# SebTanz/StochQuant

Measured on AMD Instinct MI355X. Metric: lattice-site Langevin updates/sec at 256³ fp32; achieved HBM GB/s vs peak, higher is better.
Workload: dtype fp32

## Files before the change

### stochquant_amd/build.py

```python
import argparse
import concurrent.futures as cf
import hashlib
import os
import shutil
import subprocess
import sys

PKG = os.path.dirname(os.path.abspath(__file__))
ROOT = os.path.dirname(PKG)
CSRC = os.path.join(PKG, "csrc")
OBJ = os.path.join(PKG, "_obj")
LIBDIR = os.path.join(PKG, "lib")
BINDIR = os.path.join(PKG, "bin")
LIB = os.path.join(LIBDIR, "libstochquant.so")
TAUHOST = os.path.join(BINDIR, "tauhost.o")
ROCM = os.environ.get("ROCM_PATH", "/opt/rocm")
HIPCC = os.path.join(ROCM, "bin", "hipcc")
ARCH = os.environ.get("SQ_OFFLOAD_ARCH", "gfx950")

DEVICE_SOURCES = ["sq_phi4.hip", "sq_phi4_run.hip", "sq_qm1d.hip", "sq_qm1d_ens.hip", "sq_qm1d_gs.hip", "sq_phi4_ens.hip",
                  "sq_selftest.hip", "sq_p2p.hip", "sq_fields.hip"]
HOST_SOURCES = ["sq_core.cpp", "sq_comm.cpp", "sq_phi4_create.cpp", "sq_phi4_plan.cpp", "sq_phi4_steps.cpp",
                "sq_phi4_frames.cpp", "sq_phi4_fields.cpp", "sq_qm1d_host.cpp", "sq_ens.cpp", "sq_phi4_ens.cpp",
                "sq_diag.cpp", "sq_io.cpp"]
HEADERS = ["sq_internal.h", "sq_ctx.h", "sq_rng.h", "sq_dpp.h", "sq_glibcf.h", "sq_ens.h", "sq_phi4_ens.h", "sq_qm1d_math.h"]
INCLUDES = {"sq_phi4_run.hip": ["sq_phi4.hip"], "sq_phi4_ens.hip": ["sq_phi4.hip"]}
COMMON = ["-O3", "-fPIC", "-std=c++17", "-ffp-contract=off", "-fno-slp-vectorize", "-Wall",
          "-Wno-unused-function"]


def _digest(paths, extra):
    h = hashlib.sha256()
    for p in paths:
        with open(p, "rb") as fh:
            h.update(fh.read())
    h.update(" ".join(extra).encode())
    return h.hexdigest()


def build_id(objs):
    def h(paths):
        d = hashlib.sha256()
        for p in paths:
            with open(p, "rb") as fh:
                d.update(fh.read())
        return d.hexdigest()[:16]
    phi4 = [o for o in objs if os.path.basename(o) == "sq_phi4.hip.o"]
    return f"phi4:{h(phi4)} lib:{h(objs)}"


def _run(cmd):
    r = subprocess.run(cmd, capture_output=True, text=True)
    if r.returncode != 0:
        raise RuntimeError("build failed:\n" + " ".join(cmd) + "\n" + r.stdout + r.stderr)
    return r


def build(force=False, verbose=False):
    os.makedirs(OBJ, exist_ok=True)
    os.makedirs(LIBDIR, exist_ok=True)
    os.makedirs(BINDIR, exist_ok=True)
    hdrs = [os.path.join(CSRC, h) for h in HEADERS] + [os.path.join(ROOT, "include", "stochquant.h")]
    jobs = []
    for src in DEVICE_SOURCES + HOST_SOURCES:
        s = os.path.join(CSRC, src)
        o = os.path.join(OBJ, src + ".o")
        flags = COMMON + [f"--offload-arch={ARCH}", "-x", "hip"]
        stamp = o + ".sha"
        dig = _digest([s] + [os.path.join(CSRC, d) for d in INCLUDES.get(src, [])] + hdrs, flags)
        if not force and os.path.exists(o) and os.path.exists(stamp) and open(stamp).read() == dig:
            continue
        jobs.append(([HIPCC] + flags + ["-c", s, "-o", o], stamp, dig))
    with cf.ThreadPoolExecutor(max_workers=min(8, os.cpu_count() or 4)) as ex:
        for (cmd, stamp, dig), _ in zip(jobs, ex.map(lambda j: _run(j[0]), jobs)):
            with open(stamp, "w") as fh:
                fh.write(dig)
            if verbose:
                print(" ".join(cmd))
    objs = [os.path.join(OBJ, s + ".o") for s in DEVICE_SOURCES + HOST_SOURCES]
    bid = build_id(objs)
    bid_obj = os.path.join(OBJ, "sq_build_id.cpp.o")
    bid_stamp = bid_obj + ".sha"
    if jobs or force or not os.path.exists(bid_obj) or not os.path.exists(bid_stamp) or \
            open(bid_stamp).read() != bid:
        _run([HIPCC] + COMMON + ["-x", "c++", f'-DSQ_BUILD_ID="{bid}"', "-c",
                                 os.path.join(CSRC, "sq_build_id.cpp"), "-o", bid_obj])
        with open(bid_stamp, "w") as fh:
            fh.write(bid)
        jobs.append(None)
    if jobs or force or not os.path.exists(LIB):
        _run([HIPCC, f"--offload-arch={ARCH}", "-shared", "-fPIC", "-o", LIB] + objs + [bid_obj]
             + [f"-L{ROCM}/lib", "-lrccl", f"-Wl,-rpath,{ROCM}/lib"])
    th_src = os.path.join(CSRC, "tauhost.cpp")
    if jobs or force or not os.path.exists(TAUHOST) or \
            os.path.getmtime(th_src) > os.path.getmtime(TAUHOST):
        _run(["g++", "-O2", "-std=c++17", "-Wall", "-o", TAUHOST, th_src,
              f"-L{LIBDIR}", "-lstochquant", "-Wl,-rpath,$ORIGIN/../lib", f"-Wl,-rpath,{ROCM}/lib", "-lm"])
    root_link = os.path.join(ROOT, "tauhost.o")
    try:
        if os.path.islink(root_link) or os.path.exists(root_link):
            os.remove(root_link)
        os.symlink(os.path.relpath(TAUHOST, ROOT), root_link)
    except OSError:
        shutil.copy2(TAUHOST, root_link)
    return LIB


def build_oracle(verbose=False):
    odir = os.path.join(ROOT, "oracle")
    r = subprocess.run(["make", "-C", odir, "-j4"], capture_output=True, text=True)
    if r.returncode != 0:
        raise RuntimeError("oracle build failed:\n" + r.stdout + r.stderr)
    if verbose:
        print(r.stdout)
    return os.path.join(odir, "liboracle.so")


def main(argv=None):
    ap = argparse.ArgumentParser()
    ap.add_argument("--force", action="store_true")
    ap.add_argument("-v", "--verbose", action="store_true")
    a = ap.parse_args(argv)
    print(build(force=a.force, verbose=a.verbose))
    print(build_oracle(verbose=a.verbose))


if __name__ == "__main__":
    sys.exit(main())
```

### stochquant_amd/csrc/sq_internal.h

```cpp
#pragma once
#include <hip/hip_runtime.h>
#include <stdint.h>

#include <string>

namespace sq {

int set_error(int code, const std::string &msg);

}

struct sq_ctx;

namespace sq {

struct FrameState {
    float T, V;
    int init;
    int stab_cnt;
};
int frame_state_get(const sq_ctx *c, FrameState *fs);
int frame_state_set(sq_ctx *c, const FrameState &fs);

struct FrameCtl;
struct FrameFoldArgs {
    const FrameCtl *cin;
    FrameCtl *cout;
    const unsigned long long *md;
    const unsigned int *am;
    const int *flag;
    float *rec;
    int *stable_out;
    double *dtau_out;
    const float *snap;
    int L;
};
struct RecClear {
    unsigned long long *md;
    unsigned int *am;
    int *flag;
    int n;
};
constexpr int kFoldMaxL = 64;

struct Phi4StepArgs {
    const float *in;
    float *out;
    int Lx, Ly, nz, gz;
    int zlo, zhi, zstep, zc, nzc;
    int nzr, zlen;
    int periodic;
    int nxseg, nyg, nunits;
    long long zg0;
    long long Lzg;
    float h, m2, lam6, sig, clampv;
    float sigq;
    int fin;
    uint32_t k0, k1, s_lo, s_hi;
    int *flag;
    unsigned long long *st_md;
    unsigned int *st_a;
    float *snap;
    const float *dcoef;
    int prio;
    unsigned long long *stamps;
    FrameFoldArgs fold;
    RecClear clr;
    float *buf0, *buf1, *buf2;
    const FrameCtl *tctl;
    int tk;
    int tspec;
    const unsigned int *gate;
    unsigned int gate_seq;
    int n_reg, tzc, tlen, tlo0, thi0, ntz;
    int *gate_err;
};
constexpr int kStabSlots = 32;

struct FrameCtl {
    double dtau;
    double C;
    float coef[4];
    float T, V;
    int stab_cnt;
    int adapt;
    int stable;
    int fired;
    int flag;
    int frames;
    int tri, bs, bw0, bw1, nl_odd;
};
struct FrameEndArgs {
    const FrameCtl *cin;
    FrameCtl *cout;
    const unsigned long long *md;
    const unsigned int *am;
    const int *flag;
    unsigned long long *md_next;
    unsigned int *am_next;
    int *flag_next;
    int L;
    float *rec;
    int *stable_out;
    double *dtau_out;
    float4 *dst;
    const float4 *snap;
    long long n4;
};
hipError_t phi4_frame_end_launch(const FrameEndArgs &e, hipStream_t s);
constexpr double kSqrt2Ln2 = 1.1774100225154747;

struct Phi4Geom {
    int qx;
    int r;
    int wy;
    int pf;
    int v;
};

bool phi4_tb2_supported(int Lx, int Ly);
hipError_t phi4_tb2_launch(const Phi4StepArgs &a, hipStream_t s, hipEvent_t start = nullptr,
                           hipEvent_t stop = nullptr, uint64_t *kid = nullptr);

struct Tb2RunArgs {
    unsigned int *flags;
    int *err;
    unsigned int base;
    int npairs;
    unsigned long long *stamps;
};
bool phi4_tb2_run_ok(const Phi4StepArgs &a, int dev);
hipError_t phi4_tb2_run_launch(const Phi4StepArgs &a, const Tb2RunArgs &r, hipStream_t s, hipEvent_t start = nullptr,
                               hipEvent_t stop = nullptr, uint64_t *kid = nullptr);
void phi4_run_kernel_id_name(uint64_t kid, char *name, size_t cap);

struct Tb2StageArgs {
    float *stage;
    int G;
    unsigned int *ctr;
};
bool phi4_tb2_stage_ok(const Phi4StepArgs &a, int G);
hipError_t phi4_tb2_stage_launch(const Phi4StepArgs &a, const Tb2StageArgs &g, hipStream_t s,
                                 hipEvent_t start = nullptr, hipEvent_t stop = nullptr, uint64_t *kid = nullptr);

void phi4_kernel_id_name(uint64_t kid, char *name, size_t cap);
inline unsigned phi4_kernel_id_grid(uint64_t kid) { return (unsigned)(kid >> 32); }

bool phi4_geometry(int Lx, int Ly, Phi4Geom *g);
void phi4_fill_units(Phi4StepArgs &a, const Phi4Geom &g);
hipError_t phi4_step_launch(const Phi4StepArgs &a, const Phi4Geom &g, hipStream_t s,
                            hipEvent_t start = nullptr, hipEvent_t stop = nullptr, uint64_t *kid = nullptr);
hipError_t phi4_init_hash_launch(float *slab, int Lx, int Ly, int nz, long long zg0, unsigned long long key,
                                 double amp, hipStream_t s);
hipError_t phi4_init_launch(float *slab, int Lx, int Ly, int nz, long long zg0, uint32_t k0,
                            uint32_t k1, float amp, hipStream_t s);
constexpr int kMomBlocks = 1024;
hipError_t phi4_moments_launch(const float *slab, long long n, double *acc, unsigned int *acc_max, double *part,
                               hipStream_t s);
hipError_t phi4_slices_launch(const float *slab, int Lx, int Ly, int nz, double *out,
                              hipStream_t s);

enum class P2pRed { kMaxU32, kMaxI32, kMaxU64, kMaxF64, kSumF64 };
hipError_t p2p_handshake_launch(unsigned int *up_from_dn, unsigned int *dn_from_up, const unsigned int *from_dn,
                                const unsigned int *from_up, unsigned int e, unsigned int polls, int *err,
                                hipStream_t s, const unsigned int *pre = nullptr, unsigned int pre_n = 0);
hipError_t p2p_copy2_launch(float *d0, const float *s0, float *d1, const float *s1, size_t n, hipStream_t s);
hipError_t p2p_fold_launch(const unsigned char *slots, int nranks, size_t cap, void *out, size_t n, P2pRed red,
                           hipStream_t s);

struct Qm1dState {
    double omega_in;
    double omega_out;
    double lrgVl;
    int lrgEl;
    int stable;
    int steps_done;
    int sync_error;
};

struct Qm1dArgs {
    const double *f, *x, *xx0;
    double *nf, *nx, *nxx0;
    double *fs, *xs, *ds;
    double *om;
    float *xi, *tcl;
    double *dd;
    Qm1dState *st;
    int N, pot, loops, runs;
    double a, a2, h, sig, sigw, kconst;
    uint32_t k0, k1;
    unsigned long long tick;
    int gbar;
    unsigned int bar_polls;
    int bar_skip;
    unsigned long long *dbg;
};

int qm1d_sites_per_thread(int N);
constexpr int kQm1dMaxN = 1024 * 64;
constexpr int kQm1dRegMaxN = 4096;
constexpr int kQm1dGridAux = 2048;
constexpr int kQm1dStampBlocks = kQm1dMaxN / 512;
constexpr size_t kQm1dTableCap = size_t(16) << 30;
hipError_t qm1d_frame_launch(const Qm1dArgs &a, hipStream_t s);
hipError_t qm1d_prep_launch(const Qm1dArgs &a, hipStream_t s);

struct Qm1dGsState {
    double omega_in, omega_out, lrgVl;
    int lrgEl, stable, steps_done;
    int rows_ready;
    long long consumed;
    int sync_error;
    int brk_step, brk_item;
    int pad;
};

struct Qm1dGsArgs {
    const double *f0, *x0, *xx00;
    double *nf, *nx, *nxx0;
    double *nfp;
    const double *xi;
    double *om;
    double *xc;
    void *cand;
    int *flags;
    int tag;
    double *hist;
    Qm1dGsState *st;
    int N, pot, loops, runs;
    double a, a2, h, sig, sigw, kconst;
};

constexpr int kQm1dGsMaxN = 4096;
int qm1d_gs_block(int N);
constexpr int kLcgChunks = 16384;
constexpr size_t kLcgScratch = 3 * (size_t)kLcgChunks + 1;
hipError_t qm1d_gs_lcg_launch(unsigned long long seed, int N, long long ncalls, uint32_t *w1,
                              uint32_t *w2, unsigned long long *seeds, double *xi,
                              unsigned long long *scr, hipStream_t s);
size_t qm1d_gs_cand_bytes(int loops);
hipError_t qm1d_gs_frame_launch(const Qm1dGsArgs &a, hipStream_t s);

hipError_t selftest_normals_launch(float *out, size_t nquads, unsigned long long quad0,
                                   uint32_t stream, unsigned long long step, uint32_t k0,
                                   uint32_t k1, hipStream_t s);
hipError_t selftest_dpp_launch(float *out, hipStream_t s);
hipError_t selftest_dpp_mix_launch(int mode, int blocks, int iters, unsigned *errs, float *sink, hipStream_t s);
hipError_t selftest_philox_launch(const uint32_t *ck, uint32_t *out, hipStream_t s);
hipError_t selftest_libm_launch(int fn, const float *x, float *y, long long n, hipStream_t s);
hipError_t selftest_bm_tables_launch(float *t, hipStream_t s);
hipError_t copy_launch(const float4 *in, float4 *out, size_t n4, bool nt, hipStream_t s);

}
```

### stochquant_amd/csrc/sq_phi4.hip

```cpp
#include <hip/hip_ext.h>

#include <algorithm>
#include <cstdio>
#include <cstring>

#include "sq_dpp.h"
#include "sq_internal.h"
#include "sq_rng.h"

namespace sq {

namespace {

typedef float f32x4v __attribute__((ext_vector_type(4)));

__device__ __forceinline__ float from_left_lane(float v) {
    return __builtin_bit_cast(float, __builtin_amdgcn_mov_dpp(__builtin_bit_cast(int, v), 0x13C, 0xF, 0xF, true));
}
__device__ __forceinline__ float from_right_lane(float v) {
    return __builtin_bit_cast(float, __builtin_amdgcn_mov_dpp(__builtin_bit_cast(int, v), 0x134, 0xF, 0xF, true));
}
__device__ __forceinline__ float from_left_lane_or(float v, float edge) {
    return __builtin_bit_cast(float, __builtin_amdgcn_update_dpp(__builtin_bit_cast(int, edge),
                                                                 __builtin_bit_cast(int, v), 0x138, 0xF, 0xF, false));
}
__device__ __forceinline__ float from_right_lane_or(float v, float edge) {
    return __builtin_bit_cast(float, __builtin_amdgcn_update_dpp(__builtin_bit_cast(int, edge),
                                                                 __builtin_bit_cast(int, v), 0x130, 0xF, 0xF, false));
}

__device__ __forceinline__ __amdgpu_buffer_rsrc_t plane_rsrc(const float *base, int padded,
                                                             size_t plane, uint32_t pbytes) {
    return __builtin_amdgcn_make_buffer_rsrc((void *)(base + (size_t)padded * plane), (short)0,
                                             (int)pbytes, 0x00020000);
}
template <int LAUX = 0>
__device__ __forceinline__ float4 bload4(__amdgpu_buffer_rsrc_t r, uint32_t off, uint32_t soff = 0) {
    const f32x4v v = __builtin_amdgcn_raw_buffer_load_b128(r, off, soff, LAUX);
    return make_float4(v.x, v.y, v.z, v.w);
}
template <int AUX = 0>
__device__ __forceinline__ void bstore4(__amdgpu_buffer_rsrc_t r, uint32_t off, float4 v) {
    const uint32_t soff = 0;
    const f32x4v w = {v.x, v.y, v.z, v.w};
    __builtin_amdgcn_raw_buffer_store_b128(w, r, off, soff, AUX);
}
template <int LAUX = 0>
__device__ __forceinline__ float bload1(__amdgpu_buffer_rsrc_t r, uint32_t off, uint32_t soff = 0) {
    return __builtin_bit_cast(float, __builtin_amdgcn_raw_buffer_load_b32(r, off, soff, LAUX));
}

__device__ __forceinline__ int padded_index(const Phi4StepArgs &A, int zl) {
    if (A.periodic) {
        if (zl < 0) return A.nz;
        if (zl >= A.nz) return 1;
    }
    return zl + A.gz;
}

__device__ __forceinline__ int global_z(const Phi4StepArgs &A, int zl) {
    const int Lz = (int)A.Lzg;
    int zg = (int)A.zg0 + zl;
    if (zg < 0) zg += Lz;
    else if (zg >= Lz) zg -= Lz;
    return zg;
}

template <bool NZ>
__device__ __forceinline__ float site_update(float phi, float xm, float xp, float ym, float yp,
                                             float zm, float zp, float xi, const Phi4StepArgs &A) {
    const float nb = ((xm + xp) + (ym + yp)) + (zm + zp);
    const float lap = __builtin_fmaf(-6.0f, phi, nb);
    const float g = __builtin_fmaf(A.lam6, phi * phi, A.m2);
    const float drift = __builtin_fmaf(-phi, g, lap);
    const float det = __builtin_fmaf(A.h, drift, phi);
    const float v = NZ ? __builtin_fmaf(A.sigq, xi, det) : det;
    return fmaxf(fminf(v, A.clampv), -A.clampv);
}

typedef float f32x2 __attribute__((ext_vector_type(2)));
template <bool NZ>
__device__ __forceinline__ float4 site_update4(float4 c, float lft, float rgt, float4 up, float4 dn,
                                               float4 zm, float4 zp, const f32x4n &xi,
                                               const Phi4StepArgs &A, bool fin, f32x2 m2v,
                                               float *mpre = nullptr) {
    const f32x2 c0 = {c.x, c.y}, c1 = {c.z, c.w};
    float s02, s13;
    asm("v_add_f32 %0, %1, %2" : "=v"(s02) : "v"(c.x), "v"(c.z));
    asm("v_add_f32 %0, %1, %2" : "=v"(s13) : "v"(c.y), "v"(c.w));
    const f32x2 x0 = {lft + c.y, s02}, x1 = {s13, c.z + rgt};
    const f32x2 y0 = f32x2{up.x, up.y} + f32x2{dn.x, dn.y}, y1 = f32x2{up.z, up.w} + f32x2{dn.z, dn.w};
    const f32x2 z0 = f32x2{zm.x, zm.y} + f32x2{zp.x, zp.y}, z1 = f32x2{zm.z, zm.w} + f32x2{zp.z, zp.w};
    const f32x2 nb0 = (x0 + y0) + z0, nb1 = (x1 + y1) + z1;
    const f32x2 m6 = {-6.0f, -6.0f}, l6 = {A.lam6, A.lam6}, m2 = m2v, h = {A.h, A.h};
    const f32x2 lap0 = __builtin_elementwise_fma(m6, c0, nb0), lap1 = __builtin_elementwise_fma(m6, c1, nb1);
    const f32x2 g0 = __builtin_elementwise_fma(l6, c0 * c0, m2), g1 = __builtin_elementwise_fma(l6, c1 * c1, m2);
    const f32x2 d0 = __builtin_elementwise_fma(-c0, g0, lap0), d1 = __builtin_elementwise_fma(-c1, g1, lap1);
    f32x2 v0 = __builtin_elementwise_fma(h, d0, c0), v1 = __builtin_elementwise_fma(h, d1, c1);
    if (NZ) {
        const f32x2 sg = {A.sigq, A.sigq};
        v0 = __builtin_elementwise_fma(sg, f32x2{xi.a, xi.b}, v0);
        v1 = __builtin_elementwise_fma(sg, f32x2{xi.c, xi.d}, v1);
    }
    const float cl = A.clampv;
    float4 o = make_float4(v0.x, v0.y, v1.x, v1.y);
    const float m = fmaxf(fmaxf(fmaxf(fabsf(o.x), fabsf(o.y)), fabsf(o.z)), fabsf(o.w));
    float mo = m;
    if (!fin || !(m < cl)) {
        o = make_float4(fmaxf(fminf(o.x, cl), -cl), fmaxf(fminf(o.y, cl), -cl), fmaxf(fminf(o.z, cl), -cl),
                        fmaxf(fminf(o.w, cl), -cl));
        if (mpre != nullptr) mo = fmaxf(fmaxf(fabsf(o.x), fabsf(o.y)), fmaxf(fabsf(o.z), fabsf(o.w)));
    }
    if (mpre != nullptr) *mpre = mo;
    return o;
}

struct FrameAcc {
    float m, d;
    float mw;
    float am;
};
__device__ __forceinline__ FrameAcc frame_acc() {
    return FrameAcc{-__builtin_inff(), 0.f, -__builtin_inff(), 0.f};
}

__device__ __forceinline__ float vmax(float a, float b) {
    float r;
    asm("v_max_f32 %0, %1, %2" : "=v"(r) : "v"(a), "v"(b));
    return r;
}
__device__ __forceinline__ float vmax3(float a, float b, float c) {
    float r;
    asm("v_max3_f32 %0, %1, %2, %3" : "=v"(r) : "v"(a), "v"(b), "v"(c));
    return r;
}

__device__ __forceinline__ void stab_site(FrameAcc &f, float o, float c, float xi, float sig) {
    const float dn = fabsf(__builtin_fmaf(-sig, xi, o - c));
    const float dt = vmax(f.d, dn);
    const bool gt = o > f.m, eq = o == f.m;
    const float d1 = eq ? dt : f.d;
    f.d = gt ? dn : d1;
    f.m = vmax(f.m, o);
}

template <bool NZ, bool BW = false>
__device__ __forceinline__ void frame_sites(const Phi4StepArgs &A, FrameAcc &f, const float4 &o, const float4 &c,
                                            const f32x4n &xi, float *bw = nullptr, bool pre = false,
                                            float mpre = 0.f) {
    const float mo = pre ? mpre : fmaxf(fmaxf(fabsf(o.x), fabsf(o.y)), fmaxf(fabsf(o.z), fabsf(o.w)));
    f.am = vmax(f.am, mo);
    {
        if (__ballot(mo >= f.mw) == 0ull) return;
        const float o4 = vmax(vmax3(o.x, o.y, o.z), o.w);
        if (__ballot(o4 >= f.mw) == 0ull) return;
        if constexpr (BW) {
            f.mw = vmax(f.mw, __hip_atomic_load(bw, __ATOMIC_RELAXED, __HIP_MEMORY_SCOPE_WORKGROUP));
        }
        if (!BW || __ballot(o4 >= f.mw) != 0ull) {
            const float s = NZ ? A.sigq : 0.f;
            stab_site(f, o.x, c.x, xi.a, s);
            stab_site(f, o.y, c.y, xi.b, s);
            stab_site(f, o.z, c.z, xi.c, s);
            stab_site(f, o.w, c.w, xi.d, s);
            f.mw = dpp_all_max_f(f.m);
            if (BW && (threadIdx.x & 63) == 0)
                __hip_atomic_fetch_max(bw, f.mw, __ATOMIC_RELAXED, __HIP_MEMORY_SCOPE_WORKGROUP);
        }
    }
}

__device__ __forceinline__ uint32_t ord_f32(float v) {
    const uint32_t u = __float_as_uint(v);
    return (u & 0x80000000u) ? ~u : (u | 0x80000000u);
}

__device__ __forceinline__ void frame_flush(const Phi4StepArgs &A, const FrameAcc &f, int rec, uint64_t *sk,
                                            uint32_t *sa) {
    const bool bad = f.am >= A.clampv;
    if (__ballot(bad) != 0ull && (threadIdx.x & 63) == 0) atomicOr(A.flag, 1);
    if (A.st_md == nullptr) return;
    uint64_t k = dpp_all_max_u64(((uint64_t)ord_f32(f.m) << 32) | __float_as_uint(f.d));
    uint32_t a = (uint32_t)dpp_all_max_i((int)__float_as_uint(fminf(f.am, A.clampv)));
    const int w = threadIdx.x >> 6, nw = blockDim.x >> 6;
    __syncthreads();
    if ((threadIdx.x & 63) == 0) {
        sk[w] = k;
        sa[w] = a;
    }
    __syncthreads();
    if (threadIdx.x == 0) {
        for (int i = 1; i < nw; ++i) {
            k = sk[i] > k ? sk[i] : k;
            a = sa[i] > a ? sa[i] : a;
        }
        const int slot = rec * kStabSlots + (int)(blockIdx.x % kStabSlots);
        atomicMax(A.st_md + slot, (unsigned long long)k);
        atomicMax(A.st_a + slot, a);
    }
}

__device__ __forceinline__ void frame_flush2(const Phi4StepArgs &A, const FrameAcc &f1, const FrameAcc &f2,
                                             unsigned long long *fk, uint32_t *fa) {
    const bool bad = f1.am >= A.clampv || f2.am >= A.clampv;
    if (__ballot(bad) != 0ull && (threadIdx.x & 63) == 0) atomicOr(A.flag, 1);
    if (A.st_md == nullptr) return;
    if (f1.m >= f1.mw && f1.mw > -__builtin_inff())
        atomicMax(&fk[0], ((uint64_t)ord_f32(f1.m) << 32) | __float_as_uint(f1.d));
    if (f2.m >= f2.mw && f2.mw > -__builtin_inff())
        atomicMax(&fk[1], ((uint64_t)ord_f32(f2.m) << 32) | __float_as_uint(f2.d));
    const uint32_t a1 = (uint32_t)dpp_all_max_i((int)__float_as_uint(fminf(f1.am, A.clampv)));
    const uint32_t a2 = (uint32_t)dpp_all_max_i((int)__float_as_uint(fminf(f2.am, A.clampv)));
    if ((threadIdx.x & 63) == 0) {
        atomicMax(&fa[0], a1);
        atomicMax(&fa[1], a2);
    }
    __syncthreads();
    if (threadIdx.x < 2) {
        const int slot = (int)threadIdx.x * kStabSlots + (int)(blockIdx.x % kStabSlots);
        atomicMax(A.st_md + slot, fk[threadIdx.x]);
        atomicMax(A.st_a + slot, fa[threadIdx.x]);
    }
}

__device__ __forceinline__ uint32_t uni(uint32_t v) { return __builtin_amdgcn_readfirstlane(v); }

template <int R>
__device__ __forceinline__ void philox_field(u32x4 (&c)[R], uint32_t k0, uint32_t k1) {
    const uint32_t cy = c[0].y, cz = c[0].z, cw = c[0].w;
    const uint64_t p1u = (uint64_t)kPhiloxM1 * cz;
    const uint32_t u0 = uni((uint32_t)(p1u >> 32) ^ cy ^ k0), u1 = uni((uint32_t)p1u);
    const uint32_t a0 = cw ^ k1;
    uint32_t n2[R], n3[R];
#pragma unroll
    for (int r = 0; r < R; ++r) {
        const uint64_t p0 = (uint64_t)kPhiloxM0 * c[r].x;
        n2[r] = (uint32_t)(p0 >> 32) ^ a0;
        n3[r] = (uint32_t)p0;
    }
    k0 += kPhiloxW0;
    k1 += kPhiloxW1;
    const uint64_t p0u = (uint64_t)kPhiloxM0 * u0;
    const uint32_t b0 = uni(u1 ^ k0), b2 = uni((uint32_t)(p0u >> 32) ^ k1), u3 = uni((uint32_t)p0u);
#pragma unroll
    for (int r = 0; r < R; ++r) {
        const uint64_t p1 = (uint64_t)kPhiloxM1 * n2[r];
        c[r] = u32x4{(uint32_t)(p1 >> 32) ^ b0, (uint32_t)p1, b2 ^ n3[r], u3};
    }
    k0 += kPhiloxW0;
    k1 += kPhiloxW1;
    const uint32_t d2 = uni(u3 ^ k1);
#pragma unroll
    for (int r = 0; r < R; ++r) {
        const uint64_t p0 = (uint64_t)kPhiloxM0 * c[r].x;
        const uint64_t p1 = (uint64_t)kPhiloxM1 * c[r].z;
        const uint32_t n0 = __builtin_amdgcn_bitop3_b32((uint32_t)(p1 >> 32), c[r].y, k0, 0x96);
        c[r] = u32x4{n0, (uint32_t)p1, (uint32_t)(p0 >> 32) ^ d2, (uint32_t)p0};
    }
#pragma unroll
    for (int rnd = 3; rnd < 10; ++rnd) {
        k0 += kPhiloxW0;
        k1 += kPhiloxW1;
#pragma unroll
        for (int r = 0; r < R; ++r) {
            const uint64_t p0 = (uint64_t)kPhiloxM0 * c[r].x;
            const uint64_t p1 = (uint64_t)kPhiloxM1 * c[r].z;
            const uint32_t n0 = __builtin_amdgcn_bitop3_b32((uint32_t)(p1 >> 32), c[r].y, k0, 0x96);
            const uint32_t m2 = __builtin_amdgcn_bitop3_b32((uint32_t)(p0 >> 32), c[r].w, k1, 0x96);
            c[r] = u32x4{n0, (uint32_t)p1, m2, (uint32_t)p0};
        }
    }
}

template <int R>
__device__ __forceinline__ void philox_rows(u32x4 (&c)[R], uint32_t k0, uint32_t k1) {
#pragma unroll
    for (int rnd = 0; rnd < 10; ++rnd) {
        if (rnd) {
            k0 += kPhiloxW0;
            k1 += kPhiloxW1;
        }
#pragma unroll
        for (int r = 0; r < R; ++r) {
            const uint64_t p0 = (uint64_t)kPhiloxM0 * c[r].x;
            const uint64_t p1 = (uint64_t)kPhiloxM1 * c[r].z;
            const uint32_t n0 = __builtin_amdgcn_bitop3_b32((uint32_t)(p1 >> 32), c[r].y, k0, 0x96);
            const uint32_t n2 = __builtin_amdgcn_bitop3_b32((uint32_t)(p0 >> 32), c[r].w, k1, 0x96);
            c[r] = u32x4{n0, (uint32_t)p1, n2, (uint32_t)p0};
        }
    }
}

template <int R, int V>
struct Slot {
    float4 row[R * V];
    float4 hm[V], hp[V];
};

template <int QX, int R, int V>
struct Lane {
    uint32_t voff[R * V];
    uint32_t vm[V], vp[V];
    uint32_t vl[R], vr[R];
    uint32_t qoff[R * V];
    bool rows_ok;
    int lane;
};

template <int QX, int R, int V>
__device__ __forceinline__ void load_slot(const Phi4StepArgs &A, const Lane<QX, R, V> &L,
                                          Slot<R, V> &s, int zl, bool halo, size_t plane,
                                          uint32_t pbytes) {
    const __amdgpu_buffer_rsrc_t rs = plane_rsrc(A.in, padded_index(A, zl), plane, pbytes);
#pragma unroll
    for (int k = 0; k < R * V; ++k) s.row[k] = bload4(rs, L.voff[k]);
    if (halo) {
#pragma unroll
        for (int v = 0; v < V; ++v) {
            s.hm[v] = bload4(rs, L.vm[v]);
            s.hp[v] = bload4(rs, L.vp[v]);
        }
    }
}

template <int QX, int R, int V, bool MS, bool NZ, bool PK, int SAUX, bool FR>
__device__ __forceinline__ void plane_compute(const Phi4StepArgs &A, const Lane<QX, R, V> &L,
                                              const Slot<R, V> &P, const Slot<R, V> &C,
                                              const Slot<R, V> &N, int z, size_t plane,
                                              uint32_t pbytes, uint32_t qplane, uint32_t slo, uint32_t shi,
                                              FrameAcc &fa) {
    float el[R], er[R];
    if constexpr (MS) {
        const __amdgpu_buffer_rsrc_t rs = plane_rsrc(A.in, padded_index(A, z), plane, pbytes);
#pragma unroll
        for (int r = 0; r < R; ++r) {
            el[r] = 0.f;
            er[r] = 0.f;
            if (L.lane == 0) el[r] = bload1(rs, L.vl[r]);
            if (L.lane == 63) er[r] = bload1(rs, L.vr[r]);
        }
    }
    f32x4n xi[R * V];
    if constexpr (NZ) {
        u32x4 c[R * V];
        const uint32_t qbase = (uint32_t)global_z(A, z) * qplane;
#pragma unroll
        for (int k = 0; k < R * V; ++k) c[k] = u32x4{qbase + L.qoff[k], kStreamField << 24, slo, shi};
        philox_field<R * V>(c, A.k0, A.k1);
#pragma unroll
        for (int k = 0; k < R * V; ++k) {
            box_muller_q(c[k].x, c[k].y, xi[k].a, xi[k].b);
            box_muller_q(c[k].z, c[k].w, xi[k].c, xi[k].d);
        }
    } else {
#pragma unroll
        for (int k = 0; k < R * V; ++k) xi[k] = f32x4n{0.f, 0.f, 0.f, 0.f};
    }
    float4 hmv[V], hpv[V];
#pragma unroll
    for (int v = 0; v < V; ++v) {
        hmv[v] = C.hm[v];
        hpv[v] = C.hp[v];
    }
    const __amdgpu_buffer_rsrc_t ws = plane_rsrc(A.out, A.periodic ? z + 1 : z + A.gz, plane, pbytes);
#pragma unroll
    for (int r = 0; r < R; ++r) {
        float rl[V], rr[V];
#pragma unroll
        for (int v = 0; v < V; ++v) {
            const float4 cc = C.row[r * V + v];
            if constexpr (QX == 64) {
                rl[v] = from_left_lane(cc.w);
                rr[v] = from_right_lane(cc.x);
            } else {
                const int seg = L.lane & ~(QX - 1), xq = L.lane & (QX - 1);
                rl[v] = __shfl(cc.w, seg | ((xq + QX - 1) & (QX - 1)), 64);
                rr[v] = __shfl(cc.x, seg | ((xq + 1) & (QX - 1)), 64);
            }
        }
#pragma unroll
        for (int v = 0; v < V; ++v) {
            const int k = r * V + v;
            const float4 cc = C.row[k];
            const float4 up = r > 0 ? C.row[r > 0 ? k - V : 0] : hmv[v];
            const float4 dn = r < R - 1 ? C.row[r < R - 1 ? k + V : 0] : hpv[v];
            float lft = rl[v], rgt = rr[v];
            if constexpr (V > 1) {
                if (L.lane == 0) lft = rl[(v + V - 1) % V];
                if (L.lane == 63) rgt = rr[(v + 1) % V];
            }
            if constexpr (MS) {
                if (v == 0 && L.lane == 0) lft = el[r];
                if (v == V - 1 && L.lane == 63) rgt = er[r];
            }
            float4 o;
            if constexpr (PK) {
                o = site_update4<NZ>(cc, lft, rgt, up, dn, P.row[k], N.row[k], xi[k], A, A.fin != 0,
                                     f32x2{A.m2, A.m2});
            } else {
                o.x = site_update<NZ>(cc.x, lft, cc.y, up.x, dn.x, P.row[k].x, N.row[k].x, xi[k].a, A);
                o.y = site_update<NZ>(cc.y, cc.x, cc.z, up.y, dn.y, P.row[k].y, N.row[k].y, xi[k].b, A);
                o.z = site_update<NZ>(cc.z, cc.y, cc.w, up.z, dn.z, P.row[k].z, N.row[k].z, xi[k].c, A);
                o.w = site_update<NZ>(cc.w, cc.z, rgt, up.w, dn.w, P.row[k].w, N.row[k].w, xi[k].d, A);
            }
            if constexpr (FR) frame_sites<NZ>(A, fa, o, cc, xi[k]);
            if (L.rows_ok) bstore4<SAUX>(ws, L.voff[k], o);
        }
    }
}

template <int QX, int R, int V, bool MS, bool NZ, bool PK, int SAUX, bool FR>
__device__ __forceinline__ void plane_step(const Phi4StepArgs &A, const Lane<QX, R, V> &L,
                                           const Slot<R, V> &P, const Slot<R, V> &C, Slot<R, V> &N,
                                           int z, int zend, size_t plane, uint32_t pbytes,
                                           uint32_t qplane, uint32_t slo, uint32_t shi, FrameAcc &fa) {
    load_slot<QX, R, V>(A, L, N, z + 1, z + 1 < zend, plane, pbytes);
    plane_compute<QX, R, V, MS, NZ, PK, SAUX, FR>(A, L, P, C, N, z, plane, pbytes, qplane, slo, shi, fa);
}

template <int QX, int R, int V, bool MS, bool NZ, int PF, bool FR>
__device__ __forceinline__ void unit_run(const Phi4StepArgs &A, int unit, FrameAcc &fa, uint32_t slo, uint32_t shi) {
    constexpr int RS = 64 / QX;
    const int xs = unit % A.nxseg;
    const int rest = unit / A.nxseg;
    const int yg = rest % A.nyg;
    const int zk = rest / A.nyg;
    const int zbeg = A.zlo + zk * A.zstep;
    const int zend = min(zbeg + A.zc, A.zhi);

    const int Lx = A.Lx, Ly = A.Ly;
    const size_t plane = (size_t)Lx * (size_t)Ly;
    const uint32_t pbytes = (uint32_t)(plane * sizeof(float));
    const uint32_t qplane = (uint32_t)(plane >> 2);
    Lane<QX, R, V> L;
    L.lane = threadIdx.x & 63;
    const int xq = L.lane & (QX - 1);
    const int rsid = L.lane / QX;
    const int xspan = xs * (4 * QX * V);
    const int x = xspan + 4 * xq;
    const int y0r = yg * (RS * R) + rsid * R;
    L.rows_ok = y0r < Ly;
    const int y0 = L.rows_ok ? y0r : 0;
    const int ym = y0 == 0 ? Ly - 1 : y0 - 1;
    const int yp = (y0 + R == Ly) ? 0 : y0 + R;
    const int xl = (xspan == 0 ? Lx : xspan) - 1;
    const int xr = (xspan + 4 * QX * V == Lx) ? 0 : xspan + 4 * QX * V;
#pragma unroll
    for (int r = 0; r < R; ++r) {
#pragma unroll
        for (int v = 0; v < V; ++v) {
            const int xv = x + 4 * QX * v;
            L.voff[r * V + v] = (uint32_t)(((y0 + r) * Lx + xv) * 4);
            L.qoff[r * V + v] = (uint32_t)(((y0 + r) * Lx + xv) >> 2);
        }
        L.vl[r] = (uint32_t)(((y0 + r) * Lx + xl) * 4);
        L.vr[r] = (uint32_t)(((y0 + r) * Lx + xr) * 4);
    }
#pragma unroll
    for (int v = 0; v < V; ++v) {
        L.vm[v] = (uint32_t)((ym * Lx + x + 4 * QX * v) * 4);
        L.vp[v] = (uint32_t)((yp * Lx + x + 4 * QX * v) * 4);
    }

    Slot<R, V> S0, S1, S2;
    load_slot<QX, R, V>(A, L, S0, zbeg - 1, false, plane, pbytes);
    load_slot<QX, R, V>(A, L, S1, zbeg, true, plane, pbytes);
    constexpr bool PK = PF >= 3;
    constexpr int SAUX = PF == 4 ? 2 : PF == 7 ? 17 : 0;
    for (int z = zbeg; z < zend; z += 3) {
        plane_step<QX, R, V, MS, NZ, PK, SAUX, FR>(A, L, S0, S1, S2, z, zend, plane, pbytes, qplane, slo, shi, fa);
        if (z + 1 >= zend) break;
        plane_step<QX, R, V, MS, NZ, PK, SAUX, FR>(A, L, S1, S2, S0, z + 1, zend, plane, pbytes, qplane, slo, shi, fa);
        if (z + 2 >= zend) break;
        plane_step<QX, R, V, MS, NZ, PK, SAUX, FR>(A, L, S2, S0, S1, z + 2, zend, plane, pbytes, qplane, slo, shi, fa);
    }
}

__device__ __forceinline__ uintptr_t pick_buf(const Phi4StepArgs &A, int i) {
    const uintptr_t b0 = reinterpret_cast<uintptr_t>(A.buf0), b1 = reinterpret_cast<uintptr_t>(A.buf1),
                    b2 = reinterpret_cast<uintptr_t>(A.buf2);
    return i == 0 ? b0 : (i == 1 ? b1 : b2);
}

__device__ __forceinline__ float unord_f32_dev(uint32_t o);
__device__ __forceinline__ void frame_decide(FrameCtl &c, float T, float V, int fired, int flag);

struct FrameOv {
    uintptr_t in, out, snap;
    float h, sig, sigq;
};

template <bool FR>
__device__ __forceinline__ void frame_fold(const Phi4StepArgs &A, FrameOv &ov) {
    if constexpr (FR) {
        if (A.clr.md != nullptr) {
            const int gt = (int)(blockIdx.x * blockDim.x + threadIdx.x), gs = (int)(gridDim.x * blockDim.x);
            for (int q = gt; q < A.clr.n; q += gs) {
                A.clr.md[q] = 0ull;
                A.clr.am[q] = 0u;
            }
            if (gt == 0) *A.clr.flag = 0;
        }
        if (A.fold.cin == nullptr) return;
        __shared__ unsigned long long sK[kFoldMaxL];
        __shared__ unsigned int sAm[kFoldMaxL];
        __shared__ float sCoef[3];
        __shared__ int sSt, sBuf[2];
        const int L = A.fold.L;
        for (int j = (int)threadIdx.x; j < L; j += (int)blockDim.x) {
            sK[j] = 0ull;
            sAm[j] = 0u;
        }
        __syncthreads();
        for (int q = (int)threadIdx.x; q < L * kStabSlots; q += (int)blockDim.x) {
            atomicMax(&sK[q / kStabSlots], A.fold.md[q]);
            atomicMax(&sAm[q / kStabSlots], A.fold.am[q]);
        }
        __syncthreads();
        if (threadIdx.x == 0) {
            FrameCtl c = *A.fold.cin;
            float T = c.T, V = c.V;
            int fired = -1;
            for (int j = 0; j < L; ++j) {
                const float M = unord_f32_dev((uint32_t)(sK[j] >> 32)), D = __uint_as_float((uint32_t)sK[j]);
                const float Aj = __uint_as_float(sAm[j]);
                const bool f = M > T && D > V;
                T = M;
                V = V < Aj ? Aj : V;
                if (f) {
                    fired = j;
                    break;
                }
            }
            frame_decide(c, T, V, fired, *A.fold.flag);
            sCoef[0] = c.coef[0];
            sCoef[1] = c.coef[1];
            sCoef[2] = c.coef[2];
            sSt = c.stable;
            sBuf[0] = c.bs;
            sBuf[1] = c.bw0;
            if (blockIdx.x == 0) {
                *A.fold.cout = c;
                if (A.fold.stable_out) *A.fold.stable_out = c.stable;
                if (A.fold.dtau_out) *A.fold.dtau_out = c.dtau;
            }
        }
        if (blockIdx.x == 0)
            for (int j = (int)threadIdx.x; j < L; j += (int)blockDim.x) {
                A.fold.rec[j] = unord_f32_dev((uint32_t)(sK[j] >> 32));
                A.fold.rec[L + j] = __uint_as_float((uint32_t)sK[j]);
                A.fold.rec[2 * L + j] = __uint_as_float(sAm[j]);
            }
        __syncthreads();
        const bool tri = A.buf0 != nullptr, st = sSt != 0;
        const uintptr_t snapv = reinterpret_cast<uintptr_t>(A.fold.snap) -
                                sizeof(float) * (size_t)A.gz * (size_t)A.Lx * (size_t)A.Ly;
        const uintptr_t in = tri ? pick_buf(A, sBuf[0]) : (st ? ov.in : snapv);
        const uintptr_t out = tri ? pick_buf(A, sBuf[1]) : ov.out;
        const uintptr_t sn = (!tri && !st) ? uintptr_t(0) : ov.snap;
        ov.in = in;
        ov.out = out;
        ov.snap = sn;
        ov.h = sCoef[0];
        ov.sig = sCoef[1];
        ov.sigq = sCoef[2];
    }
}

struct TriCheck {
    uintptr_t in, out;
    bool on;
};

template <bool FR, bool SPEC = false>
__device__ __forceinline__ Phi4StepArgs frame_args(const Phi4StepArgs &A0, TriCheck *chk = nullptr) {
    if constexpr (FR) {
        FrameOv ov{reinterpret_cast<uintptr_t>(A0.in), reinterpret_cast<uintptr_t>(A0.out),
                   reinterpret_cast<uintptr_t>(A0.snap), A0.h, A0.sig, A0.sigq};
        if (A0.dcoef != nullptr) {
            ov.h = A0.dcoef[0];
            ov.sig = A0.dcoef[1];
            ov.sigq = A0.dcoef[2];
        }
        if (A0.tctl != nullptr) {
            const int bs = A0.tctl->bs, bw0 = A0.tctl->bw0, bw1 = A0.tctl->bw1;
            const int bi = A0.tk == 0 ? bs : ((A0.tk & 1) ? bw0 : bw1);
            const int bo = A0.tk == 0 ? bw0 : ((A0.tk & 1) ? bw1 : bw0);
            const uintptr_t in = pick_buf(A0, bi), out = pick_buf(A0, bo);
            if (SPEC && A0.tspec != 0) {
                chk->in = in;
                chk->out = out;
                chk->on = true;
            } else {
                ov.in = in;
                ov.out = out;
            }
        }
        frame_fold<FR>(A0, ov);
        Phi4StepArgs A = A0;
        A.in = reinterpret_cast<const float *>(ov.in);
        A.out = reinterpret_cast<float *>(ov.out);
        A.snap = reinterpret_cast<float *>(ov.snap);
        A.h = ov.h;
        A.sig = ov.sig;
        A.sigq = ov.sigq;
        return A;
    } else {
        return A0;
    }
}

template <int QX, int R, int V, bool MS, bool NZ, int PF, bool FR>
__global__ __launch_bounds__(256) void phi4_step_kernel(const Phi4StepArgs A0) {
    const Phi4StepArgs A = frame_args<FR>(A0);
    const int nb = gridDim.x, b = blockIdx.x;
    const int lb = (nb & 7) == 0 ? (b & 7) * (nb >> 3) + (b >> 3) : b;
    const int unit = __builtin_amdgcn_readfirstlane(lb * 4 + (int)(threadIdx.x >> 6));
    FrameAcc fa = frame_acc();
    if (unit < A.nunits) unit_run<QX, R, V, MS, NZ, PF, FR>(A, unit, fa, A.s_lo, A.s_hi);
    if constexpr (FR) {
        __shared__ uint64_t sk[4];
        __shared__ uint32_t sa[4];
        frame_flush(A, fa, 0, sk, sa);
    }
}

__device__ __forceinline__ void block_stamp(const Phi4StepArgs &A, int at) {
    const unsigned long long rt = __builtin_amdgcn_s_memrealtime(), ct = __builtin_amdgcn_s_memtime();
    A.stamps[2 * blockIdx.x + at] = rt;
    A.stamps[2 * gridDim.x + 2 * blockIdx.x + at] = ct;
}
__device__ __forceinline__ void block_end_stamp(const Phi4StepArgs &A) {
    if (A.stamps == nullptr) return;
    __syncthreads();
    if (threadIdx.x == 0) block_stamp(A, 1);
}

struct PrioQ {
    int t0, t1, t2;
    __device__ __forceinline__ PrioQ(int z0, int span)
        : t0(z0 - 1 + (span + 3) / 4), t1(z0 - 1 + (2 * span + 3) / 4), t2(z0 - 1 + (3 * span + 3) / 4) {}
    __device__ __forceinline__ int q(int p) const { return (p >= t0) + (p >= t1) + (p >= t2); }
};

__device__ __forceinline__ void prio_by_progress(int q) {
    switch (q) {
    case 0: __builtin_amdgcn_s_setprio(3); break;
    case 1: __builtin_amdgcn_s_setprio(2); break;
    case 2: __builtin_amdgcn_s_setprio(1); break;
    default: __builtin_amdgcn_s_setprio(0); break;
    }
}

struct TbBlock {
    int yb, xs, z0, z1;
    bool gated;
};
template <bool WIDE>
__device__ __forceinline__ TbBlock tb_block(const Phi4StepArgs &A, int b, int nb) {
    TbBlock t;
    t.gated = A.gate != nullptr && b >= A.n_reg;
    const int nbr = A.gate != nullptr ? A.n_reg : nb;
    const int lb = t.gated ? b - A.n_reg : ((nbr & 7) == 0 ? (b & 7) * (nbr >> 3) + (b >> 3) : b);
    t.yb = lb % A.nyg;
    const int rest = lb / A.nyg;
    t.xs = WIDE ? rest % A.nxseg : 0;
    const int zk = WIDE ? rest / A.nxseg : rest;
    if (t.gated) {
        const int r0 = zk >= A.ntz ? A.thi0 : A.tlo0;
        t.z0 = r0 + (zk % A.ntz) * A.tzc;
        t.z1 = min(t.z0 + A.tzc, r0 + A.tlen);
    } else {
        const int r0 = A.zlo + (zk / A.nzr) * A.zstep;
        t.z0 = r0 + (zk % A.nzr) * A.zc;
        t.z1 = min(t.z0 + A.zc, r0 + A.zlen);
    }
    return t;
}

constexpr unsigned int kGateSpinMax = 1u << 24;
__device__ __forceinline__ bool tb_gate_wait(const Phi4StepArgs &A) {
    __shared__ int s_gate_ok;
    if (threadIdx.x == 0) {
        unsigned int n = 0;
        int ok = 1;
        while (__hip_atomic_load(A.gate, __ATOMIC_ACQUIRE, __HIP_MEMORY_SCOPE_AGENT) < A.gate_seq) {
            __builtin_amdgcn_s_sleep(2);
            if (++n >= kGateSpinMax) {
                if (A.gate_err) __hip_atomic_fetch_or(A.gate_err, 1, __ATOMIC_RELAXED, __HIP_MEMORY_SCOPE_AGENT);
                ok = 0;
                break;
            }
        }
        s_gate_ok = ok;
    }
    __syncthreads();
    __builtin_amdgcn_fence(__ATOMIC_ACQUIRE, "agent");
    return s_gate_ok != 0;
}

constexpr int kTbRows = 8;
constexpr int kTbWaves = kTbRows + 2;

__device__ __forceinline__ int tb_pidx(const Phi4StepArgs &A, int zl) {
    if (A.periodic) zl = zl < 0 ? zl + A.nz : (zl >= A.nz ? zl - A.nz : zl);
    return zl + A.gz;
}

template <bool NZ>
__device__ __forceinline__ f32x4n tb_noise(const Phi4StepArgs &A, uint32_t qz, uint32_t qoff, uint32_t slo,
                                           uint32_t shi) {
    f32x4n xi;
    if constexpr (NZ) {
        u32x4 c[1];
        c[0] = u32x4{qz + qoff, kStreamField << 24, slo, shi};
        philox_field<1>(c, A.k0, A.k1);
        box_muller_q(c[0].x, c[0].y, xi.a, xi.b);
        box_muller_q(c[0].z, c[0].w, xi.c, xi.d);
    } else {
        xi = f32x4n{0.f, 0.f, 0.f, 0.f};
    }
    return xi;
}

struct TbIn {
    float4 row, hm, hp;
};

typedef float f32x4v __attribute__((ext_vector_type(4)));

struct TbCtx {
    size_t plane;
    uint32_t pbytes, qplane;
    __amdgpu_buffer_rsrc_t rin, rout;
    uint32_t voff, vm, vp, vex, vx2, qoff;
    uint32_t slo, shi, slo1, shi1;
    uint32_t qwrap;
    f32x2 m2v;
    int swrap_at;
    int z0, z1, w, lane;
    bool outw;
    int snapw;
    __amdgpu_buffer_rsrc_t rstg;
    int stg_g, stg_hi;
};

struct TbRun {
    uint32_t snext, scur;
    uint32_t qz, qzm;
};

__device__ __forceinline__ float tb_site(float phi, float xm, float xp, float ym, float yp, float zm, float zp,
                                         float xi, const Phi4StepArgs &A, bool nz) {
    const float nb = ((xm + xp) + (ym + yp)) + (zm + zp);
    const float lap = __builtin_fmaf(-6.0f, phi, nb);
    const float g = __builtin_fmaf(A.lam6, phi * phi, A.m2);
    const float drift = __builtin_fmaf(-phi, g, lap);
    const float det = __builtin_fmaf(A.h, drift, phi);
    const float v = nz ? __builtin_fmaf(A.sigq, xi, det) : det;
    return fmaxf(fminf(v, A.clampv), -A.clampv);
}

__device__ __forceinline__ void tb_wait_nbrs(const int *prog, int w, int need) {
    const int wl = w > 0 ? w - 1 : w + 1, wr = w < kTbWaves - 1 ? w + 1 : w - 1;
    for (;;) {
        const int a = __hip_atomic_load(&prog[wl], __ATOMIC_ACQUIRE, __HIP_MEMORY_SCOPE_WORKGROUP);
        const int b = __hip_atomic_load(&prog[wr], __ATOMIC_ACQUIRE, __HIP_MEMORY_SCOPE_WORKGROUP);
        if (__builtin_amdgcn_readfirstlane(min(a, b)) >= need) break;
        __builtin_amdgcn_s_sleep(1);
    }
}

template <bool NZ, bool WIDE, bool FR, bool WH, int J, bool P2 = false, int LAUX = 0, bool STG = false>
__device__ __forceinline__ void tb_plane(const Phi4StepArgs &A, const TbCtx &K, TbRun &R, int p, const TbIn &I0,
                                         const TbIn &I1, TbIn &I2, const float4 &T0, const float4 &T1, float4 &T2,
                                         float4 (*lds)[kTbWaves][64], float (*tx)[kTbWaves][2], FrameAcc &f1,
                                         FrameAcc &f2, float *bmx, int *prog = nullptr) {
    constexpr int sl = J, sp = (J + 2) % 3;
    __amdgpu_buffer_rsrc_t rs, rc;
    uint32_t ss = 0, sc = 0;
    if constexpr (WH) {
        rs = rc = K.rin;
        ss = R.snext;
        sc = R.scur;
    } else {
        rs = plane_rsrc(A.in, tb_pidx(A, p + 1), K.plane, K.pbytes);
        rc = plane_rsrc(A.in, tb_pidx(A, p), K.plane, K.pbytes);
    }
    if (!WIDE || K.w < kTbWaves) {
        I2.row = bload4<LAUX>(rs, K.voff, ss);
        I2.hm = bload4<LAUX>(rs, K.vm, ss);
        I2.hp = bload4<LAUX>(rs, K.vp, ss);
        float ex = 0.f;
        if constexpr (WIDE) ex = bload1(rc, K.vex, sc);
        const f32x4n xa = tb_noise<NZ>(A, R.qz, K.qoff, K.slo, K.shi);
        float lft, rgt;
        if constexpr (WIDE) {
            lft = from_left_lane_or(I1.row.w, ex);
            rgt = from_right_lane_or(I1.row.x, ex);
        } else {
            lft = from_left_lane(I1.row.w);
            rgt = from_right_lane(I1.row.x);
        }
        float mp1;
        T2 = site_update4<NZ>(I1.row, lft, rgt, I1.hm, I1.hp, I0.row, I2.row, xa, A, A.fin != 0, K.m2v, &mp1);
        if constexpr (FR) {
            if (K.outw && p >= K.z0 && p < K.z1) frame_sites<NZ, true>(A, f1, T2, I1.row, xa, bmx, true, mp1);
            if (K.snapw != 0 && p + 1 >= K.z0 && p + 1 < K.z1)
                __builtin_nontemporal_store(
                    (f32x4v){I2.row.x, I2.row.y, I2.row.z, I2.row.w},
                    reinterpret_cast<f32x4v *>(reinterpret_cast<char *>(A.snap) + (size_t)(p + 1) * K.pbytes + K.voff));
        }
        if constexpr (P2) tb_wait_nbrs(prog, K.w, p - 1);
        lds[sl][K.w][K.lane] = T2;
    } else {
        I2.row.x = bload1(rs, K.voff, ss);
        const float xm = bload1(rc, K.vex, sc), xp = bload1(rc, K.vx2, sc), ym = bload1(rc, K.vm, sc),
                    yp = bload1(rc, K.vp, sc);
        const f32x4n n = tb_noise<NZ>(A, R.qz, K.qoff, K.slo, K.shi);
        const float xi = K.lane >= 8 ? n.a : n.d;
        const float t = tb_site(I1.row.x, xm, xp, ym, yp, I0.row.x, I2.row.x, xi, A, NZ);
        if (K.lane < 16) tx[sl][(K.lane & 7) + 1][K.lane >> 3] = t;
    }
    if constexpr (P2) {
        if (K.lane == 0) __hip_atomic_store(&prog[K.w], p, __ATOMIC_RELEASE, __HIP_MEMORY_SCOPE_WORKGROUP);
    } else {
        __syncthreads();
    }
    if (K.outw && p > K.z0) {
        const f32x4n xb = tb_noise<NZ>(A, R.qzm, K.qoff, K.slo1, K.shi1);
        const float4 up = lds[sp][K.w - 1][K.lane], dn = lds[sp][K.w + 1][K.lane];
        float lft, rgt;
        if constexpr (WIDE) {
            const float2 e = *reinterpret_cast<const float2 *>(&tx[sp][K.w][0]);
            lft = from_left_lane_or(T1.w, e.x);
            rgt = from_right_lane_or(T1.x, e.y);
        } else {
            lft = from_left_lane(T1.w);
            rgt = from_right_lane(T1.x);
        }
        float mp2;
        const float4 o = site_update4<NZ>(T1, lft, rgt, up, dn, T0, T2, xb, A, true, K.m2v, &mp2);
        if constexpr (FR) frame_sites<NZ, true>(A, f2, o, T1, xb, bmx + 1, true, mp2);
        if constexpr (WH) {
            bstore4<17>(K.rout, K.voff + (uint32_t)(p - 1 + A.gz) * K.pbytes, o);
            if constexpr (STG) {
                const int q = p - 1;
                if (q < K.stg_g) bstore4<17>(K.rstg, K.voff + (uint32_t)q * K.pbytes, o);
                if (q >= K.stg_hi) bstore4<17>(K.rstg, K.voff + (uint32_t)(q - K.stg_hi + K.stg_g) * K.pbytes, o);
            }
        } else {
            const __amdgpu_buffer_rsrc_t ws = plane_rsrc(A.out, p - 1 + A.gz, K.plane, K.pbytes);
            bstore4<17>(ws, K.voff, o);
        }
    }
    R.qzm = R.qz;
    const uint32_t q = R.qz + K.qplane;
    R.qz = q == K.qwrap ? 0u : q;
    if constexpr (WH) {
        R.scur = R.snext;
        R.snext = p == K.swrap_at ? (uint32_t)A.gz * K.pbytes : R.snext + K.pbytes;
    }
}

template <bool NZ, bool WIDE, int WPE, bool FR, bool WH, bool P2 = false>
__global__ __launch_bounds__((kTbWaves + (WIDE ? 1 : 0)) * 64)
__attribute__((amdgpu_waves_per_eu(WPE))) void phi4_tb2_kernel(const Phi4StepArgs A0) {
    static_assert(!P2 || !WIDE, "neighbour sync: 256-site rows");
    TriCheck chk{0, 0, false};
    Phi4StepArgs A = frame_args<FR, true>(A0, &chk);
    const int nb = gridDim.x, b = blockIdx.x;
    if (A.stamps != nullptr && threadIdx.x == 0) block_stamp(A, 0);
    const TbBlock tbk = tb_block<WIDE>(A, b, nb);
    const int yb = tbk.yb, xs = tbk.xs;
    const int Lx = A.Lx, Ly = A.Ly;
    const int x0 = 256 * xs;
    TbCtx K;
    K.w = __builtin_amdgcn_readfirstlane((int)(threadIdx.x >> 6));
    K.lane = threadIdx.x & 63;
    K.outw = K.w >= 1 && K.w <= kTbRows;
    K.z0 = tbk.z0;
    const int z1 = tbk.z1;
    K.snapw = __builtin_amdgcn_readfirstlane((FR && A.snap != nullptr && K.outw) ? 1 : 0);
    K.z1 = z1;
    K.plane = (size_t)Lx * (size_t)Ly;
    K.pbytes = (uint32_t)(K.plane * sizeof(float));
    K.qplane = (uint32_t)(K.plane >> 2);
    if constexpr (WH) {
        const int nbytes = (int)((uint32_t)(A.nz + 2 * A.gz) * K.pbytes);
        K.rin = __builtin_amdgcn_make_buffer_rsrc((void *)A.in, (short)0, nbytes, 0x00020000);
        K.rout = __builtin_amdgcn_make_buffer_rsrc((void *)A.out, (short)0, nbytes, 0x00020000);
    }
    K.qwrap = (uint32_t)A.Lzg * K.qplane;
    K.m2v = f32x2{A.m2, A.m2};
    asm volatile("" : "+v"(K.m2v));
    K.swrap_at = A.periodic ? A.nz - 2 : INT_MIN;
    const unsigned long long s0 = ((unsigned long long)A.s_hi << 32) | A.s_lo, s1 = s0 + 1;
    K.slo = (uint32_t)s0;
    K.shi = (uint32_t)(s0 >> 32);
    K.slo1 = (uint32_t)s1;
    K.shi1 = (uint32_t)(s1 >> 32);
    const int xl = (x0 == 0 ? Lx : x0) - 1, xr = x0 + 256 == Lx ? 0 : x0 + 256;
    auto wrapy = [Ly](int y) { return y < 0 ? y + Ly : (y >= Ly ? y - Ly : y); };
    if (!WIDE || K.w < kTbWaves) {
        const int y = wrapy(yb * kTbRows - 1 + K.w);
        const int ym = wrapy(y - 1), yp = wrapy(y + 1);
        K.voff = (uint32_t)((y * Lx + x0 + 4 * K.lane) * 4);
        K.vm = (uint32_t)((ym * Lx + x0 + 4 * K.lane) * 4);
        K.vp = (uint32_t)((yp * Lx + x0 + 4 * K.lane) * 4);
        K.vex = (uint32_t)((y * Lx + (K.lane == 63 ? xr : xl)) * 4);
        K.vx2 = 0;
        K.qoff = (uint32_t)((y * Lx + x0 + 4 * K.lane) >> 2);
    } else {
        const int l = K.lane < 16 ? K.lane : 0;
        const int y = wrapy(yb * kTbRows + (l & 7)), ym = wrapy(y - 1), yp = wrapy(y + 1);
        const int xe = (l >> 3) ? xr : xl;
        const int xem = xe == 0 ? Lx - 1 : xe - 1, xep = xe == Lx - 1 ? 0 : xe + 1;
        K.voff = (uint32_t)((y * Lx + xe) * 4);
        K.vex = (uint32_t)((y * Lx + xem) * 4);
        K.vx2 = (uint32_t)((y * Lx + xep) * 4);
        K.vm = (uint32_t)((ym * Lx + xe) * 4);
        K.vp = (uint32_t)((yp * Lx + xe) * 4);
        K.qoff = (uint32_t)((y * Lx + xe) >> 2);
    }
    __shared__ float4 lds[3][kTbWaves][64];
    __shared__ float tx[WIDE ? 3 : 1][kTbWaves][2];

    if (tbk.gated && !tb_gate_wait(A)) return;
    TbIn I0, I1, I2;
    auto prologue = [&]() {
        const __amdgpu_buffer_rsrc_t r0 = plane_rsrc(A.in, tb_pidx(A, K.z0 - 2), K.plane, K.pbytes);
        const __amdgpu_buffer_rsrc_t r1 = plane_rsrc(A.in, tb_pidx(A, K.z0 - 1), K.plane, K.pbytes);
        if (!WIDE || K.w < kTbWaves) {
            I0.row = bload4(r0, K.voff);
            I0.hm = I0.hp = I0.row;
            I1.row = bload4(r1, K.voff);
            I1.hm = bload4(r1, K.vm);
            I1.hp = bload4(r1, K.vp);
        } else {
            I0.row = make_float4(bload1(r0, K.voff), 0.f, 0.f, 0.f);
            I1.row = make_float4(bload1(r1, K.voff), 0.f, 0.f, 0.f);
            I0.hm = I0.hp = I1.hm = I1.hp = I0.row;
        }
    };
    prologue();
    if constexpr (FR) {
        if (chk.on && (chk.in != reinterpret_cast<uintptr_t>(A.in) || chk.out != reinterpret_cast<uintptr_t>(A.out))) {
            A.in = reinterpret_cast<const float *>(chk.in);
            A.out = reinterpret_cast<float *>(chk.out);
            if constexpr (WH) {
                const int nbytes = (int)((uint32_t)(A.nz + 2 * A.gz) * K.pbytes);
                K.rin = __builtin_amdgcn_make_buffer_rsrc((void *)A.in, (short)0, nbytes, 0x00020000);
                K.rout = __builtin_amdgcn_make_buffer_rsrc((void *)A.out, (short)0, nbytes, 0x00020000);
            }
            prologue();
        }
    }
    float4 T0 = make_float4(0.f, 0.f, 0.f, 0.f), T1 = T0, T2 = T0;
    FrameAcc f1 = frame_acc(), f2 = frame_acc();
    __shared__ float bmx[2];
    __shared__ unsigned long long fk[2];
    __shared__ uint32_t fa[2];
    if constexpr (FR) {
        if (threadIdx.x < 2) {
            bmx[threadIdx.x] = -__builtin_inff();
            fk[threadIdx.x] = 0ull;
            fa[threadIdx.x] = 0u;
        }
        __syncthreads();
    }
    TbRun R;
    R.scur = (uint32_t)tb_pidx(A, K.z0 - 1) * K.pbytes;
    R.snext = (uint32_t)tb_pidx(A, K.z0) * K.pbytes;
    R.qz = (uint32_t)global_z(A, K.z0 - 1) * K.qplane;
    R.qzm = 0;
    __shared__ int prog[P2 ? kTbWaves : 1];
    if constexpr (P2) {
        if (threadIdx.x < kTbWaves) prog[threadIdx.x] = K.z0 - 2;
        __syncthreads();
    }
    const PrioQ pq(K.z0, z1 - K.z0 + 2);
    for (int p = K.z0 - 1; p <= z1; p += 3) {
        if (A.prio) prio_by_progress(pq.q(p));
        tb_plane<NZ, WIDE, FR, WH, 0, P2>(A, K, R, p, I0, I1, I2, T0, T1, T2, lds, tx, f1, f2, bmx, prog);
        if (p + 1 > z1) break;
        tb_plane<NZ, WIDE, FR, WH, 1, P2>(A, K, R, p + 1, I1, I2, I0, T1, T2, T0, lds, tx, f1, f2, bmx, prog);
        if (p + 2 > z1) break;
        tb_plane<NZ, WIDE, FR, WH, 2, P2>(A, K, R, p + 2, I2, I0, I1, T2, T0, T1, lds, tx, f1, f2, bmx, prog);
    }
    if constexpr (FR) frame_flush2(A, f1, f2, fk, fa);
    block_end_stamp(A);
}

constexpr int kTpRows = kTbWaves + 2;
constexpr uint32_t kTpOob = 0x80000000u;

struct TpRun {
    uint32_t s2, s1;
    uint32_t qz, qzm;
};

template <bool WH>
__device__ __forceinline__ void tp_advance(const Phi4StepArgs &A, const TbCtx &K, TpRun &R, int k) {
    R.qzm = R.qz;
    const uint32_t q = R.qz + K.qplane;
    R.qz = q == K.qwrap ? 0u : q;
    if constexpr (WH) {
        R.s1 = R.s2;
        R.s2 = k + 3 == K.swrap_at ? (uint32_t)A.gz * K.pbytes : R.s2 + K.pbytes;
    }
}

template <bool NZ, bool WIDE, bool FR, bool WH, int J>
__device__ __forceinline__ void tp_row(const Phi4StepArgs &A, const TbCtx &K, TpRun &R, int k, bool xrow,
                                       uint32_t vxr, int xslot, float4 (&I)[4], float4 (&T)[4], float4 (&X)[2],
                                       float (&E)[2], float4 (*in_lds)[kTpRows][64], float4 (*t_lds)[kTbWaves][64],
                                       float (*tx)[kTbWaves][2], FrameAcc &f1, FrameAcc &f2, float *bmx) {
    constexpr int im = J, ic = (J + 1) & 3, ip = (J + 2) & 3, in2 = (J + 3) & 3;
    constexpr int tc = J, tm = (J + 3) & 3, tmm = (J + 2) & 3;
    constexpr int sc = J & 1, sn = (J + 1) & 1;
    const bool more = k < K.z1;
    __amdgpu_buffer_rsrc_t r2, r1;
    uint32_t o2 = 0, o1 = 0;
    if constexpr (WH) {
        r2 = r1 = K.rin;
        o2 = R.s2;
        o1 = R.s1;
    } else {
        r2 = plane_rsrc(A.in, tb_pidx(A, k + 2), K.plane, K.pbytes);
        r1 = plane_rsrc(A.in, tb_pidx(A, k + 1), K.plane, K.pbytes);
    }
    I[in2] = bload4(r2, more ? K.voff : kTpOob, o2);
    X[sc] = bload4(r2, more ? vxr : kTpOob, o2);
    if constexpr (WIDE) E[sn] = bload1(r1, more ? K.vex : kTpOob, o1);
    in_lds[sn][K.w + 1][K.lane] = I[ip];
    if (xrow) in_lds[sn][xslot][K.lane] = X[sn];
    if constexpr (FR) {
        const bool sv = K.snapw != 0 && k + 1 >= K.z0 && k + 1 < K.z1;
        bstore4<2>(plane_rsrc(A.snap, k + 1, K.plane, K.pbytes), sv ? K.voff : kTpOob, I[ip]);
    }
    const f32x4n xa = tb_noise<NZ>(A, R.qz, K.qoff, K.slo, K.shi);
    const float4 up = in_lds[sc][K.w][K.lane], dn = in_lds[sc][K.w + 2][K.lane];
    float lft, rgt;
    if constexpr (WIDE) {
        lft = from_left_lane_or(I[ic].w, E[sc]);
        rgt = from_right_lane_or(I[ic].x, E[sc]);
    } else {
        lft = from_left_lane(I[ic].w);
        rgt = from_right_lane(I[ic].x);
    }
    float mp1;
    T[tc] = site_update4<NZ>(I[ic], lft, rgt, up, dn, I[im], I[ip], xa, A, A.fin != 0, K.m2v, &mp1);
    if constexpr (FR) {
        if (K.outw && k >= K.z0 && k < K.z1) frame_sites<NZ, true>(A, f1, T[tc], I[ic], xa, bmx, true, mp1);
    }
    t_lds[sc][K.w][K.lane] = T[tc];
    const bool bw = K.outw && k > K.z0;
    float4 o = T[tc];
    if (bw) {
        const f32x4n xb = tb_noise<NZ>(A, R.qzm, K.qoff, K.slo1, K.shi1);
        const float4 bu = t_lds[sn][K.w - 1][K.lane], bd = t_lds[sn][K.w + 1][K.lane];
        float bl, br;
        if constexpr (WIDE) {
            const float2 e = *reinterpret_cast<const float2 *>(&tx[sn][K.w][0]);
            bl = from_left_lane_or(T[tm].w, e.x);
            br = from_right_lane_or(T[tm].x, e.y);
        } else {
            bl = from_left_lane(T[tm].w);
            br = from_right_lane(T[tm].x);
        }
        float mp2;
        o = site_update4<NZ>(T[tm], bl, br, bu, bd, T[tmm], T[tc], xb, A, true, K.m2v, &mp2);
        if constexpr (FR) frame_sites<NZ, true>(A, f2, o, T[tm], xb, bmx + 1, true, mp2);
    }
    if constexpr (WH) {
        bstore4<17>(K.rout, bw ? K.voff + (uint32_t)(k - 1 + A.gz) * K.pbytes : kTpOob, o);
    } else {
        const __amdgpu_buffer_rsrc_t ws = plane_rsrc(A.out, k - 1 + A.gz, K.plane, K.pbytes);
        bstore4<17>(ws, bw ? K.voff : kTpOob, o);
    }
    __syncthreads();
    tp_advance<WH>(A, K, R, k);
}

template <bool NZ, bool WH, int J>
__device__ __forceinline__ void tp_xhalo(const Phi4StepArgs &A, const TbCtx &K, TpRun &R, int k, float (&C)[4],
                                         float4 (&NB)[2], float (*tx)[kTbWaves][2]) {
    constexpr int im = J, ic = (J + 1) & 3, ip = (J + 2) & 3, in2 = (J + 3) & 3;
    constexpr int sc = J & 1, sn = (J + 1) & 1;
    {
        const bool more = k < K.z1;
        __amdgpu_buffer_rsrc_t r2, r1;
        uint32_t o2 = 0, o1 = 0;
        if constexpr (WH) {
            r2 = r1 = K.rin;
            o2 = R.s2;
            o1 = R.s1;
        } else {
            r2 = plane_rsrc(A.in, tb_pidx(A, k + 2), K.plane, K.pbytes);
            r1 = plane_rsrc(A.in, tb_pidx(A, k + 1), K.plane, K.pbytes);
        }
        C[in2] = bload1(r2, more ? K.voff : kTpOob, o2);
        NB[sn] = make_float4(bload1(r1, more ? K.vex : kTpOob, o1), bload1(r1, more ? K.vx2 : kTpOob, o1),
                             bload1(r1, more ? K.vm : kTpOob, o1), bload1(r1, more ? K.vp : kTpOob, o1));
    }
    const f32x4n n = tb_noise<NZ>(A, R.qz, K.qoff, K.slo, K.shi);
    const float xi = K.lane >= 8 ? n.a : n.d;
    const float t = tb_site(C[ic], NB[sc].x, NB[sc].y, NB[sc].z, NB[sc].w, C[im], C[ip], xi, A, NZ);
    if (K.lane < 16) tx[sc][(K.lane & 7) + 1][K.lane >> 3] = t;
    __syncthreads();
    tp_advance<WH>(A, K, R, k);
}

template <bool NZ, bool WIDE, int WPE, bool FR, bool WH>
__global__ __launch_bounds__((kTbWaves + (WIDE ? 1 : 0)) * 64)
__attribute__((amdgpu_waves_per_eu(WPE))) void phi4_tb2p_kernel(const Phi4StepArgs A0) {
    const Phi4StepArgs A = frame_args<FR>(A0);
    const int nb = gridDim.x, b = blockIdx.x;
    if (A.stamps != nullptr && threadIdx.x == 0) block_stamp(A, 0);
    const TbBlock tbk = tb_block<WIDE>(A, b, nb);
    const int yb = tbk.yb, xs = tbk.xs;
    const int Lx = A.Lx, Ly = A.Ly;
    const int x0 = 256 * xs;
    TbCtx K;
    K.w = __builtin_amdgcn_readfirstlane((int)(threadIdx.x >> 6));
    K.lane = threadIdx.x & 63;
    K.outw = K.w >= 1 && K.w <= kTbRows;
    K.snapw = __builtin_amdgcn_readfirstlane((FR && A.snap != nullptr && K.outw) ? 1 : 0);
    K.z0 = tbk.z0;
    K.z1 = tbk.z1;
    K.plane = (size_t)Lx * (size_t)Ly;
    K.pbytes = (uint32_t)(K.plane * sizeof(float));
    K.qplane = (uint32_t)(K.plane >> 2);
    if constexpr (WH) {
        const int nbytes = (int)((uint32_t)(A.nz + 2 * A.gz) * K.pbytes);
        K.rin = __builtin_amdgcn_make_buffer_rsrc((void *)A.in, (short)0, nbytes, 0x00020000);
        K.rout = __builtin_amdgcn_make_buffer_rsrc((void *)A.out, (short)0, nbytes, 0x00020000);
    }
    K.qwrap = (uint32_t)A.Lzg * K.qplane;
    K.m2v = f32x2{A.m2, A.m2};
    asm volatile("" : "+v"(K.m2v));
    K.swrap_at = A.periodic ? A.nz : INT_MIN;
    const unsigned long long s0 = ((unsigned long long)A.s_hi << 32) | A.s_lo, s1 = s0 + 1;
    K.slo = (uint32_t)s0;
    K.shi = (uint32_t)(s0 >> 32);
    K.slo1 = (uint32_t)s1;
    K.shi1 = (uint32_t)(s1 >> 32);
    const int xl = (x0 == 0 ? Lx : x0) - 1, xr = x0 + 256 == Lx ? 0 : x0 + 256;
    auto wrapy = [Ly](int y) { return y < 0 ? y + Ly : (y >= Ly ? y - Ly : y); };
    const bool xw = WIDE && K.w == kTbWaves;
    const bool xrow = K.w == 0 || K.w == kTbWaves - 1;
    const int xslot = K.w == 0 ? 0 : kTpRows - 1;
    uint32_t vxr = kTpOob;
    if (!xw) {
        const int y = wrapy(yb * kTbRows - 1 + K.w);
        const int yx = wrapy(K.w == 0 ? y - 1 : y + 1);
        K.voff = (uint32_t)((y * Lx + x0 + 4 * K.lane) * 4);
        if (xrow) vxr = (uint32_t)((yx * Lx + x0 + 4 * K.lane) * 4);
        K.vm = K.vp = 0;
        K.vex = (uint32_t)((y * Lx + (K.lane == 63 ? xr : xl)) * 4);
        K.vx2 = 0;
        K.qoff = (uint32_t)((y * Lx + x0 + 4 * K.lane) >> 2);
    } else {
        const int l = K.lane < 16 ? K.lane : 0;
        const int y = wrapy(yb * kTbRows + (l & 7)), ym = wrapy(y - 1), yp = wrapy(y + 1);
        const int xe = (l >> 3) ? xr : xl;
        const int xem = xe == 0 ? Lx - 1 : xe - 1, xep = xe == Lx - 1 ? 0 : xe + 1;
        K.voff = (uint32_t)((y * Lx + xe) * 4);
        K.vex = (uint32_t)((y * Lx + xem) * 4);
        K.vx2 = (uint32_t)((y * Lx + xep) * 4);
        K.vm = (uint32_t)((ym * Lx + xe) * 4);
        K.vp = (uint32_t)((yp * Lx + xe) * 4);
        K.qoff = (uint32_t)((y * Lx + xe) >> 2);
    }
    __shared__ float4 in_lds[2][kTpRows][64];
    __shared__ float4 t_lds[2][kTbWaves][64];
    __shared__ float tx[WIDE ? 2 : 1][kTbWaves][2];

    if (tbk.gated && !tb_gate_wait(A)) return;
    const __amdgpu_buffer_rsrc_t p0 = plane_rsrc(A.in, tb_pidx(A, K.z0 - 2), K.plane, K.pbytes);
    const __amdgpu_buffer_rsrc_t p1 = plane_rsrc(A.in, tb_pidx(A, K.z0 - 1), K.plane, K.pbytes);
    const __amdgpu_buffer_rsrc_t p2 = plane_rsrc(A.in, tb_pidx(A, K.z0), K.plane, K.pbytes);
    __shared__ float bmx[2];
    __shared__ unsigned long long fk[2];
    __shared__ uint32_t fa[2];
    if constexpr (FR) {
        if (threadIdx.x < 2) {
            bmx[threadIdx.x] = -__builtin_inff();
            fk[threadIdx.x] = 0ull;
            fa[threadIdx.x] = 0u;
        }
    }
    FrameAcc f1 = frame_acc(), f2 = frame_acc();
    TpRun R;
    R.s1 = (uint32_t)tb_pidx(A, K.z0) * K.pbytes;
    R.s2 = (uint32_t)tb_pidx(A, K.z0 + 1) * K.pbytes;
    R.qz = (uint32_t)global_z(A, K.z0 - 1) * K.qplane;
    R.qzm = 0;
    const int z1 = K.z1;
    if (!xw) {
        float4 I[4], T[4], X[2];
        float E[2] = {0.f, 0.f};
        I[0] = bload4(p0, K.voff);
        I[1] = bload4(p1, K.voff);
        I[2] = bload4(p2, K.voff);
        X[0] = bload4(p1, vxr);
        X[1] = bload4(p2, vxr);
        if constexpr (WIDE) E[0] = bload1(p1, K.vex);
        in_lds[0][K.w + 1][K.lane] = I[1];
        if (xrow) in_lds[0][xslot][K.lane] = X[0];
        T[0] = T[1] = T[2] = T[3] = make_float4(0.f, 0.f, 0.f, 0.f);
        __syncthreads();
        const PrioQ pq(K.z0, z1 - K.z0 + 2);
        for (int k = K.z0 - 1; k <= z1; k += 4) {
            if (A.prio) prio_by_progress(pq.q(k));
            tp_row<NZ, WIDE, FR, WH, 0>(A, K, R, k, xrow, vxr, xslot, I, T, X, E, in_lds, t_lds, tx, f1, f2, bmx);
            if (k + 1 > z1) break;
            tp_row<NZ, WIDE, FR, WH, 1>(A, K, R, k + 1, xrow, vxr, xslot, I, T, X, E, in_lds, t_lds, tx, f1, f2, bmx);
            if (k + 2 > z1) break;
            tp_row<NZ, WIDE, FR, WH, 2>(A, K, R, k + 2, xrow, vxr, xslot, I, T, X, E, in_lds, t_lds, tx, f1, f2, bmx);
            if (k + 3 > z1) break;
            tp_row<NZ, WIDE, FR, WH, 3>(A, K, R, k + 3, xrow, vxr, xslot, I, T, X, E, in_lds, t_lds, tx, f1, f2, bmx);
        }
    } else {
        float C[4];
        float4 NB[2];
        C[0] = bload1(p0, K.voff);
        C[1] = bload1(p1, K.voff);
        C[2] = bload1(p2, K.voff);
        NB[0] = make_float4(bload1(p1, K.vex), bload1(p1, K.vx2), bload1(p1, K.vm), bload1(p1, K.vp));
        __syncthreads();
        const PrioQ pq(K.z0, z1 - K.z0 + 2);
        for (int k = K.z0 - 1; k <= z1; k += 4) {
            if (A.prio) prio_by_progress(pq.q(k));
            tp_xhalo<NZ, WH, 0>(A, K, R, k, C, NB, tx);
            if (k + 1 > z1) break;
            tp_xhalo<NZ, WH, 1>(A, K, R, k + 1, C, NB, tx);
            if (k + 2 > z1) break;
            tp_xhalo<NZ, WH, 2>(A, K, R, k + 2, C, NB, tx);
            if (k + 3 > z1) break;
            tp_xhalo<NZ, WH, 3>(A, K, R, k + 3, C, NB, tx);
        }
    }
    if constexpr (FR) frame_flush2(A, f1, f2, fk, fa);
    block_end_stamp(A);
}

__global__ __launch_bounds__(256) void phi4_init_kernel(float *slab, int Lx, int Ly, int nz,
                                                        long long zg0, uint32_t k0, uint32_t k1,
                                                        float amp) {
    const size_t plane = (size_t)Lx * Ly;
    const size_t nq = (size_t)nz * plane / 4;
    const uint64_t q0 = (uint64_t)zg0 * (uint64_t)(plane >> 2);
    for (size_t q = (size_t)blockIdx.x * blockDim.x + threadIdx.x; q < nq;
         q += (size_t)gridDim.x * blockDim.x) {
        const f32x4n n = normals4(q0 + q, kStreamInit, 0u, 0u, k0, k1);
        *reinterpret_cast<float4 *>(slab + 4 * q) = make_float4(amp * n.a, amp * n.b, amp * n.c, amp * n.d);
    }
}

__device__ __forceinline__ double wave_sum(double v) {
#pragma unroll
    for (int o = 32; o > 0; o >>= 1) v += __shfl_xor(v, o, 64);
    return v;
}
__device__ __forceinline__ float wave_max(float v) {
#pragma unroll
    for (int o = 32; o > 0; o >>= 1) v = fmaxf(v, __shfl_xor(v, o, 64));
    return v;
}

constexpr int kEndChunk = 512;

__device__ __forceinline__ float unord_f32_dev(uint32_t o) {
    return __uint_as_float((o & 0x80000000u) ? (o & 0x7FFFFFFFu) : ~o);
}

__device__ __forceinline__ void frame_decide(FrameCtl &c, float T, float V, int fired, int flag) {
    const int st = (flag == 0 && fired < 0) ? 1 : 0;
    c.T = T;
    c.V = V;
    c.fired = fired;
    c.flag = flag;
    c.stable = st;
    c.frames += 1;
    if (c.adapt) {
        if (st) {
            if (c.stab_cnt > 10) {
                c.stab_cnt = 0;
                c.dtau /= 0.950;
            }
            c.stab_cnt += 1;
        } else {
            c.dtau *= 0.950;
            c.stab_cnt = 0;
        }
    }
    const float hf = (float)c.dtau;
    c.coef[0] = hf;
    c.coef[1] = (float)(__builtin_sqrt(2.0 * (double)hf) * c.C);
    c.coef[2] = (float)(__builtin_sqrt(2.0 * (double)hf) * c.C * kSqrt2Ln2);
    if (c.tri) {
        const int fin = c.nl_odd ? c.bw0 : c.bw1;
        const int third = 3 - c.bs - fin;
        const int nbs = st ? fin : c.bs, nbw1 = st ? c.bs : fin;
        c.bs = nbs;
        c.bw0 = third;
        c.bw1 = nbw1;
    }
}

__global__ __launch_bounds__(256) void phi4_frame_end_kernel(FrameEndArgs E) {
    __shared__ float sM[kEndChunk], sD[kEndChunk], sA[kEndChunk];
    __shared__ float sT, sV;
    __shared__ int sFired;
    const bool b0 = blockIdx.x == 0;
    if (threadIdx.x == 0) {
        sT = E.cin->T;
        sV = E.cin->V;
        sFired = -1;
    }
    for (int j0 = 0; j0 < E.L; j0 += kEndChunk) {
        const int n = min(kEndChunk, E.L - j0);
        __syncthreads();
        for (int j = threadIdx.x; j < n; j += blockDim.x) {
            unsigned long long k = 0;
            unsigned int a = 0;
            const size_t q0 = (size_t)(j0 + j) * kStabSlots;
            for (int i = 0; i < kStabSlots; ++i) {
                const unsigned long long mk = E.md[q0 + i];
                const unsigned int ma = E.am[q0 + i];
                k = k < mk ? mk : k;
                a = a < ma ? ma : a;
            }
            sM[j] = unord_f32_dev((uint32_t)(k >> 32));
            sD[j] = __uint_as_float((uint32_t)k);
            sA[j] = __uint_as_float(a);
            if (b0) {
                E.rec[j0 + j] = sM[j];
                E.rec[E.L + j0 + j] = sD[j];
                E.rec[2 * E.L + j0 + j] = sA[j];
            }
        }
        __syncthreads();
        if (threadIdx.x == 0 && sFired < 0) {
            float T = sT, V = sV;
            for (int j = 0; j < n; ++j) {
                const bool f = sM[j] > T && sD[j] > V;
                T = sM[j];
                V = V < sA[j] ? sA[j] : V;
                if (f) {
                    sFired = j0 + j;
                    break;
                }
            }
            sT = T;
            sV = V;
        }
    }
    __syncthreads();
    const int st = (*E.flag == 0 && sFired < 0) ? 1 : 0;
    if (b0) {
        if (threadIdx.x == 0) {
            FrameCtl c = *E.cin;
            frame_decide(c, sT, sV, sFired, *E.flag);
            *E.cout = c;
            if (E.stable_out) *E.stable_out = st;
            if (E.dtau_out) *E.dtau_out = c.dtau;
            *E.flag_next = 0;
        }
        for (long long q = threadIdx.x; q < (long long)E.L * kStabSlots; q += blockDim.x) {
            E.md_next[q] = 0;
            E.am_next[q] = 0;
        }
    }
    if (st) return;
    for (long long i = (long long)blockIdx.x * blockDim.x + threadIdx.x; i < E.n4;
         i += (long long)gridDim.x * blockDim.x)
        E.dst[i] = E.snap[i];
}

__global__ __launch_bounds__(256) void phi4_moments_kernel(const float *p, long long n4, double *part) {
    double s1 = 0, s2 = 0;
    float mx = 0, mp = -__builtin_inff();
    const float4 *q = reinterpret_cast<const float4 *>(p);
    for (long long i = (long long)blockIdx.x * blockDim.x + threadIdx.x; i < n4;
         i += (long long)gridDim.x * blockDim.x) {
        const float4 v = q[i];
        s1 += (double)v.x + (double)v.y + (double)v.z + (double)v.w;
        s2 += (double)v.x * v.x + (double)v.y * v.y + (double)v.z * v.z + (double)v.w * v.w;
        mx = fmaxf(mx, fmaxf(fmaxf(fabsf(v.x), fabsf(v.y)), fmaxf(fabsf(v.z), fabsf(v.w))));
        mp = fmaxf(mp, fmaxf(fmaxf(v.x, v.y), fmaxf(v.z, v.w)));
    }
    __shared__ double sh1[4], sh2[4];
    __shared__ float shm[4], shp[4];
    s1 = wave_sum(s1);
    s2 = wave_sum(s2);
    mx = wave_max(mx);
    mp = wave_max(mp);
    const int w = threadIdx.x >> 6;
    if ((threadIdx.x & 63) == 0) {
        sh1[w] = s1;
        sh2[w] = s2;
        shm[w] = mx;
        shp[w] = mp;
    }
    __syncthreads();
    if (threadIdx.x == 0) {
        double t1 = 0, t2 = 0;
        float tm = 0, tp = -__builtin_inff();
        for (int k = 0; k < (int)(blockDim.x >> 6); ++k) {
            t1 += sh1[k];
            t2 += sh2[k];
            tm = fmaxf(tm, shm[k]);
            tp = fmaxf(tp, shp[k]);
        }
        double *q = part + 4 * (size_t)blockIdx.x;
        q[0] = t1;
        q[1] = t2;
        q[2] = (double)tm;
        q[3] = (double)tp;
    }
}

__global__ __launch_bounds__(256) void phi4_moments_final_kernel(const double *part, int nb, double *acc,
                                                                 unsigned int *acc_max) {
    double s1 = 0, s2 = 0, mx = 0, mp = -__builtin_inf();
    for (int b = threadIdx.x; b < nb; b += blockDim.x) {
        const double *q = part + 4 * (size_t)b;
        s1 += q[0];
        s2 += q[1];
        mx = fmax(mx, q[2]);
        mp = fmax(mp, q[3]);
    }
    __shared__ double sh[4][4];
    s1 = wave_sum(s1);
    s2 = wave_sum(s2);
#pragma unroll
    for (int o = 32; o > 0; o >>= 1) {
        mx = fmax(mx, __shfl_xor(mx, o, 64));
        mp = fmax(mp, __shfl_xor(mp, o, 64));
    }
    const int w = threadIdx.x >> 6;
    if ((threadIdx.x & 63) == 0) {
        sh[w][0] = s1;
        sh[w][1] = s2;
        sh[w][2] = mx;
        sh[w][3] = mp;
    }
    __syncthreads();
    if (threadIdx.x == 0) {
        double t1 = 0, t2 = 0, tm = 0, tp = -__builtin_inf();
        for (int k = 0; k < (int)(blockDim.x >> 6); ++k) {
            t1 += sh[k][0];
            t2 += sh[k][1];
            tm = fmax(tm, sh[k][2]);
            tp = fmax(tp, sh[k][3]);
        }
        acc[0] = t1;
        acc[1] = t2;
        acc_max[0] = __float_as_uint((float)tm);
        acc_max[1] = ord_f32((float)tp);
    }
}

__global__ __launch_bounds__(256) void phi4_slices_kernel(const float *slab, long long plane4,
                                                          double *out) {
    const float4 *q = reinterpret_cast<const float4 *>(slab) + (size_t)blockIdx.x * plane4;
    double s = 0;
    for (long long i = threadIdx.x; i < plane4; i += blockDim.x) {
        const float4 v = q[i];
        s += ((double)v.x + (double)v.y) + ((double)v.z + (double)v.w);
    }
    __shared__ double sh[4];
    s = wave_sum(s);
    if ((threadIdx.x & 63) == 0) sh[threadIdx.x >> 6] = s;
    __syncthreads();
    if (threadIdx.x == 0) out[blockIdx.x] = (sh[0] + sh[1]) + (sh[2] + sh[3]);
}

}

#ifndef SQ_PHI4_KERNELS_ONLY
bool phi4_geometry(int Lx, int Ly, Phi4Geom *g) {
    if (Lx <= 0 || Ly <= 0 || (Lx & 3)) return false;
    int qx;
    if (Lx % 256 == 0) qx = 64;
    else if (Lx < 256 && Lx >= 8 && 64 % (Lx / 4) == 0) qx = Lx / 4;
    else return false;
    const int rs = 64 / qx;
    const int v = (qx == 64 && Lx % 512 == 0) ? 2 : 1;
    const int pf = qx == 64 ? 7 : 1;
    const bool narrow = Lx <= 256;
    const int rcand[3] = {narrow ? 1 : 2, narrow ? 2 : 4, narrow ? 4 : 1};
    for (int r : rcand) {
        if (Ly % (rs * r) == 0) {
            *g = Phi4Geom{qx, r, rs * r, pf, v};
            return true;
        }
    }
    for (int r : rcand) {
        if (Ly % r == 0) {
            *g = Phi4Geom{qx, r, rs * r, pf, v};
            return true;
        }
    }
    return false;
}

void phi4_fill_units(Phi4StepArgs &a, const Phi4Geom &g) {
    a.nxseg = a.Lx / (4 * g.qx * g.v);
    a.nyg = (a.Ly + g.wy - 1) / g.wy;
    a.nunits = a.nxseg * a.nyg * a.nzc;
}

template <int QX, int R, int V, bool MS, bool NZ, int PF, bool FR>
static hipError_t launch_fr(const Phi4StepArgs &a, dim3 grid, hipStream_t s, hipEvent_t e0, hipEvent_t e1) {
    if (e0 != nullptr || e1 != nullptr)
        hipExtLaunchKernelGGL((phi4_step_kernel<QX, R, V, MS, NZ, PF, FR>), grid, dim3(256), 0, s, e0, e1, 0, a);
    else
        hipLaunchKernelGGL((phi4_step_kernel<QX, R, V, MS, NZ, PF, FR>), grid, dim3(256), 0, s, a);
    return hipGetLastError();
}

template <int QX, int R, int V, bool MS, bool NZ, int PF>
static hipError_t launch_pf(const Phi4StepArgs &a, dim3 grid, hipStream_t s, hipEvent_t e0,
                            hipEvent_t e1) {
    if (a.flag != nullptr && (a.st_md == nullptr || a.st_a == nullptr))
        return hipErrorInvalidValue;
    return a.flag != nullptr ? launch_fr<QX, R, V, MS, NZ, PF, true>(a, grid, s, e0, e1)
                             : launch_fr<QX, R, V, MS, NZ, PF, false>(a, grid, s, e0, e1);
}

template <int QX, int R, int V, bool MS>
static hipError_t launch_v(const Phi4StepArgs &a, int pf, bool nz, dim3 grid, hipStream_t s,
                           hipEvent_t e0, hipEvent_t e1) {
    if constexpr (QX == 64) {
        if (pf == 3)
            return nz ? launch_pf<QX, R, V, MS, true, 3>(a, grid, s, e0, e1)
                      : launch_pf<QX, R, V, MS, false, 3>(a, grid, s, e0, e1);
        if (pf == 4)
            return nz ? launch_pf<QX, R, V, MS, true, 4>(a, grid, s, e0, e1)
                      : launch_pf<QX, R, V, MS, false, 4>(a, grid, s, e0, e1);
        if (pf == 7)
            return nz ? launch_pf<QX, R, V, MS, true, 7>(a, grid, s, e0, e1)
                      : launch_pf<QX, R, V, MS, false, 7>(a, grid, s, e0, e1);
    }
    return nz ? launch_pf<QX, R, V, MS, true, 1>(a, grid, s, e0, e1)
              : launch_pf<QX, R, V, MS, false, 1>(a, grid, s, e0, e1);
}

template <int QX, int V, bool MS>
static hipError_t launch_r(const Phi4StepArgs &a, const Phi4Geom &g, dim3 grid, hipStream_t s,
                           hipEvent_t e0, hipEvent_t e1) {
    const bool nz = a.sig != 0.0f;
    switch (g.r) {
    case 4: return launch_v<QX, 4, V, MS>(a, g.pf, nz, grid, s, e0, e1);
    case 2: return launch_v<QX, 2, V, MS>(a, g.pf, nz, grid, s, e0, e1);
    default: return launch_v<QX, 1, V, MS>(a, g.pf, nz, grid, s, e0, e1);
    }
}

static uint64_t kid_pack(int fam, bool nz, bool wide, int e, bool fr, bool wh, bool p2, int qx, int r, int v,
                         int pf, unsigned threads) {
    return (uint64_t)fam | (uint64_t)nz << 2 | (uint64_t)wide << 3 | (uint64_t)(e & 15) << 4 | (uint64_t)fr << 8 |
           (uint64_t)wh << 9 | (uint64_t)p2 << 10 | (uint64_t)(qx & 255) << 11 | (uint64_t)(r & 15) << 19 |
           (uint64_t)(v & 3) << 23 | (uint64_t)(pf & 15) << 25 | (uint64_t)threads << 32;
}

void phi4_kernel_id_name(uint64_t k, char *name, size_t cap) {
    const int fam = (int)(k & 3);
    auto b = [&](int bit) { return ((k >> bit) & 1) ? "true" : "false"; };
    const int e = (int)((k >> 4) & 15), qx = (int)((k >> 11) & 255), r = (int)((k >> 19) & 15),
              v = (int)((k >> 23) & 3), pf = (int)((k >> 25) & 15);
    if (fam == 0)
        snprintf(name, cap, "phi4_step_kernel<%d, %d, %d, %s, %s, %d, %s>", qx, r, v, b(3), b(2), pf, b(8));
    else if (fam == 1)
        snprintf(name, cap, "phi4_tb2_kernel<%s, %s, %d, %s, %s, %s>", b(2), b(3), e, b(8), b(9), b(10));
    else
        snprintf(name, cap, "phi4_tb2p_kernel<%s, %s, %d, %s, %s>", b(2), b(3), e, b(8), b(9));
}

hipError_t phi4_step_launch(const Phi4StepArgs &a, const Phi4Geom &g, hipStream_t s, hipEvent_t e0,
                            hipEvent_t e1, uint64_t *kid) {
    if (a.nunits <= 0) return hipSuccess;
    const dim3 grid((unsigned)((a.nunits + 3) / 4));
    const bool ms = a.nxseg > 1;
    if (kid != nullptr) {
        const bool q64 = g.qx == 64;
        const int r = g.r == 4 ? 4 : g.r == 2 ? 2 : 1;
        const int pf = q64 && (g.pf == 3 || g.pf == 4 || g.pf == 7) ? g.pf : 1;
        *kid = kid_pack(0, a.sig != 0.0f, q64 && ms, 0, a.flag != nullptr, false, false, g.qx, r,
                        q64 && g.v == 2 ? 2 : 1, pf, grid.x * 256u);
    }
    switch (g.qx) {
    case 64:
        if (g.v == 2) return ms ? launch_r<64, 2, true>(a, g, grid, s, e0, e1) : launch_r<64, 2, false>(a, g, grid, s, e0, e1);
        return ms ? launch_r<64, 1, true>(a, g, grid, s, e0, e1) : launch_r<64, 1, false>(a, g, grid, s, e0, e1);
    case 32: return launch_r<32, 1, false>(a, g, grid, s, e0, e1);
    case 16: return launch_r<16, 1, false>(a, g, grid, s, e0, e1);
    case 8: return launch_r<8, 1, false>(a, g, grid, s, e0, e1);
    case 4: return launch_r<4, 1, false>(a, g, grid, s, e0, e1);
    case 2: return launch_r<2, 1, false>(a, g, grid, s, e0, e1);
    default: return hipErrorInvalidValue;
    }
}

bool phi4_tb2_supported(int Lx, int Ly) { return Lx % 256 == 0 && Ly % kTbRows == 0; }

static bool tb2_sync_p2p() {
    const char *e = getenv("SQ_TB2_SYNC");
    return e != nullptr && strcmp(e, "p2p") == 0;
}

hipError_t phi4_tb2_launch(const Phi4StepArgs &a, hipStream_t s, hipEvent_t e0, hipEvent_t e1, uint64_t *kid) {
    if (!phi4_tb2_supported(a.Lx, a.Ly) || a.nunits <= 0 || a.nxseg != a.Lx / 256 || a.nyg != a.Ly / kTbRows ||
        a.nzr < 1 || a.nzc % a.nzr != 0 || a.nunits != a.nxseg * a.nyg * a.nzc || a.zlen < 1 ||
        (long long)a.zc * a.nzr < a.zlen)
        return hipErrorInvalidValue;
    const int nr = a.nzc / a.nzr, last_end = a.zlo + (nr - 1) * a.zstep + a.zlen;
    if (nr > 1 && a.zstep < a.zlen) return hipErrorInvalidValue;
    if (a.periodic ? (a.nz < 2 || a.zlo != 0 || a.zlen != a.nz || nr != 1)
                   : (a.zlo - 2 < -a.gz || last_end + 2 > a.nz + a.gz))
        return hipErrorInvalidValue;
    unsigned grid_n = (unsigned)a.nunits;
    if (a.gate != nullptr) {
        if (a.n_reg != a.nunits || a.tzc < 1 || a.tlen < 1 || a.ntz != (a.tlen + a.tzc - 1) / a.tzc ||
            a.tlo0 - 2 < -a.gz || a.tlo0 + a.tlen + 2 > a.nz + a.gz || a.thi0 - 2 < -a.gz ||
            a.thi0 + a.tlen + 2 > a.nz + a.gz || a.periodic)
            return hipErrorInvalidValue;
        grid_n += (unsigned)(a.nxseg * a.nyg * 2 * a.ntz);
    }
    const bool wide = a.nxseg > 1;
    const dim3 grid(grid_n), block((kTbWaves + (wide ? 1 : 0)) * 64);
    const bool nz = a.sig != 0.0f;
    static const int wpe = getenv("SQ_TB2_WPE") ? atoi(getenv("SQ_TB2_WPE")) : 6;
    const bool fr = a.flag != nullptr;
    if (fr && (a.st_md == nullptr || a.st_a == nullptr)) return hipErrorInvalidValue;
    const void *fn;
    const bool wh = (long long)(a.nz + 2 * a.gz) * a.Lx * a.Ly * 4 < (1ll << 31);
    const char *pe = getenv("SQ_TB2_PIPE");
    const bool pipe = pe ? atoi(pe) != 0 : wide;
#define SQ_TB2K(N, W, E, F, H) (pipe ? (const void *)&phi4_tb2p_kernel<N, W, E, F, H> \
                                     : (const void *)&phi4_tb2_kernel<N, W, E, F, H>)
#define SQ_TB2F(N, W, E, F) (wh ? SQ_TB2K(N, W, E, F, true) : SQ_TB2K(N, W, E, F, false))
#define SQ_TB2(N, W, E) (fr ? SQ_TB2F(N, W, E, true) : SQ_TB2F(N, W, E, false))
    if (wide && wpe == 6)
        fn = nz ? SQ_TB2(true, true, 6) : SQ_TB2(false, true, 6);
    else if (wide)
        fn = nz ? SQ_TB2(true, true, 1) : SQ_TB2(false, true, 1);
    else if (fr && !pipe && tb2_sync_p2p())
        fn = nz ? (wh ? (const void *)&phi4_tb2_kernel<true, false, 6, true, true, true>
                      : (const void *)&phi4_tb2_kernel<true, false, 6, true, false, true>)
                : (wh ? (const void *)&phi4_tb2_kernel<false, false, 6, true, true, true>
                      : (const void *)&phi4_tb2_kernel<false, false, 6, true, false, true>);
    else if (fr)
        fn = nz ? SQ_TB2F(true, false, 6, true) : SQ_TB2F(false, false, 6, true);
    else if (!pipe && tb2_sync_p2p())
        fn = nz ? (wh ? (const void *)&phi4_tb2_kernel<true, false, 1, false, true, true>
                      : (const void *)&phi4_tb2_kernel<true, false, 1, false, false, true>)
                : (wh ? (const void *)&phi4_tb2_kernel<false, false, 1, false, true, true>
                      : (const void *)&phi4_tb2_kernel<false, false, 1, false, false, true>);
    else
        fn = nz ? SQ_TB2F(true, false, 1, false) : SQ_TB2F(false, false, 1, false);
#undef SQ_TB2
#undef SQ_TB2F
#undef SQ_TB2K
    if (kid != nullptr) {
        const bool p2 = !wide && !pipe && tb2_sync_p2p();
        const int e = wide ? (wpe == 6 ? 6 : 1) : (fr ? 6 : 1);
        *kid = kid_pack(pipe && !p2 ? 2 : 1, nz, wide, e, fr, wh, p2, 0, 0, 0, 0, grid.x * block.x);
    }
    Phi4StepArgs q = a;
    static const int prio = getenv("SQ_TB2_PRIO") ? atoi(getenv("SQ_TB2_PRIO")) : 1;
    q.prio = prio;
    void *args[] = {&q};
    if (e0 != nullptr || e1 != nullptr) return hipExtLaunchKernel(fn, grid, block, args, 0, s, e0, e1, 0);
    return hipLaunchKernel(fn, grid, block, args, 0, s);
}

hipError_t phi4_init_launch(float *slab, int Lx, int Ly, int nz, long long zg0, uint32_t k0,
                            uint32_t k1, float amp, hipStream_t s) {
    const size_t nq = (size_t)nz * Lx * Ly / 4;
    const unsigned grid = (unsigned)std::min<size_t>((nq + 255) / 256, 8192);
    hipLaunchKernelGGL(phi4_init_kernel, dim3(grid), dim3(256), 0, s, slab, Lx, Ly, nz, zg0, k0, k1,
                       amp);
    return hipGetLastError();
}

hipError_t phi4_frame_end_launch(const FrameEndArgs &e, hipStream_t s) {
    if (e.L < 1 || !e.cin || !e.cout || e.cin == e.cout || !e.md || !e.am || !e.flag || !e.md_next || !e.am_next ||
        !e.flag_next || e.md == e.md_next || !e.rec || (e.n4 > 0 && (!e.dst || !e.snap)))
        return hipErrorInvalidValue;
    const unsigned grid = (unsigned)std::max<long long>(1, std::min<long long>((e.n4 + 1023) / 1024, 512));
    FrameEndArgs q = e;
    hipLaunchKernelGGL(phi4_frame_end_kernel, dim3(grid), dim3(256), 0, s, q);
    return hipGetLastError();
}

hipError_t phi4_moments_launch(const float *slab, long long n, double *acc, unsigned int *acc_max, double *part,
                               hipStream_t s) {
    const long long n4 = n / 4;
    const unsigned grid = (unsigned)std::max<long long>(1, std::min<long long>((n4 + 255) / 256, kMomBlocks));
    hipLaunchKernelGGL(phi4_moments_kernel, dim3(grid), dim3(256), 0, s, slab, n4, part);
    hipLaunchKernelGGL(phi4_moments_final_kernel, dim3(1), dim3(256), 0, s, (const double *)part, (int)grid, acc,
                       acc_max);
    return hipGetLastError();
}

hipError_t phi4_slices_launch(const float *slab, int Lx, int Ly, int nz, double *out,
                              hipStream_t s) {
    hipLaunchKernelGGL(phi4_slices_kernel, dim3((unsigned)nz), dim3(256), 0, s, slab,
                       (long long)Lx * Ly / 4, out);
    return hipGetLastError();
}

#endif
}
```

### stochquant_amd/csrc/sq_phi4_run.hip

```cpp
#define SQ_PHI4_KERNELS_ONLY
#include "sq_phi4.hip"

namespace sq {

namespace {

constexpr unsigned int kRunSpinMax = 1u << 20;
constexpr int kRunErrBit = 4;

__device__ __forceinline__ bool run_wait(const Tb2RunArgs &R, int lb, int nyg, int nzc, unsigned int need) {
    int nbr[8];
    {
        const int yb = lb % nyg, zk = lb / nyg;
        int k = 0;
#pragma unroll
        for (int dz = -1; dz <= 1; ++dz)
#pragma unroll
            for (int dy = -1; dy <= 1; ++dy) {
                if (dz == 0 && dy == 0) continue;
                const int zz = zk + dz < 0 ? zk + dz + nzc : (zk + dz >= nzc ? zk + dz - nzc : zk + dz);
                const int yy = yb + dy < 0 ? yb + dy + nyg : (yb + dy >= nyg ? yb + dy - nyg : yb + dy);
                nbr[k++] = zz * nyg + yy;
            }
    }
    for (unsigned int n = 0;; ++n) {
        bool ok = true;
#pragma unroll
        for (int k = 0; k < 8; ++k)
            ok &= (int)(__hip_atomic_load(R.flags + nbr[k], __ATOMIC_RELAXED, __HIP_MEMORY_SCOPE_AGENT) - need) >= 0;
        if (ok) return true;
        if (n >= kRunSpinMax || __hip_atomic_load(R.err, __ATOMIC_RELAXED, __HIP_MEMORY_SCOPE_AGENT) != 0) {
            __hip_atomic_fetch_or(R.err, kRunErrBit, __ATOMIC_RELAXED, __HIP_MEMORY_SCOPE_AGENT);
            return false;
        }
        __builtin_amdgcn_s_sleep(1);
    }
}

template <bool NZ, int LAUX>
__global__ __launch_bounds__(kTbWaves * 64) __attribute__((amdgpu_waves_per_eu(1)))
void phi4_tb2_run_kernel(const Phi4StepArgs A0, const Tb2RunArgs R0) {
    Phi4StepArgs A = A0;
    const int nb = gridDim.x, b = blockIdx.x;
    const TbBlock tbk = tb_block<false>(A, b, nb);
    const int lb = (nb & 7) == 0 ? (b & 7) * (nb >> 3) + (b >> 3) : b;
    const int Lx = A.Lx, Ly = A.Ly;
    TbCtx K;
    K.w = __builtin_amdgcn_readfirstlane((int)(threadIdx.x >> 6));
    K.lane = threadIdx.x & 63;
    K.outw = K.w >= 1 && K.w <= kTbRows;
    K.z0 = tbk.z0;
    K.z1 = tbk.z1;
    K.snapw = 0;
    K.plane = (size_t)Lx * (size_t)Ly;
    K.pbytes = (uint32_t)(K.plane * sizeof(float));
    K.qplane = (uint32_t)(K.plane >> 2);
    K.qwrap = (uint32_t)A.Lzg * K.qplane;
    K.m2v = f32x2{A.m2, A.m2};
    asm volatile("" : "+v"(K.m2v));
    K.swrap_at = A.nz - 2;
    {
        auto wrapy = [Ly](int y) { return y < 0 ? y + Ly : (y >= Ly ? y - Ly : y); };
        const int y = wrapy(tbk.yb * kTbRows - 1 + K.w);
        const int ym = wrapy(y - 1), yp = wrapy(y + 1);
        K.voff = (uint32_t)((y * Lx + 4 * K.lane) * 4);
        K.vm = (uint32_t)((ym * Lx + 4 * K.lane) * 4);
        K.vp = (uint32_t)((yp * Lx + 4 * K.lane) * 4);
        K.vex = 0;
        K.vx2 = 0;
        K.qoff = (uint32_t)((y * Lx + 4 * K.lane) >> 2);
    }
    __shared__ float4 lds[3][kTbWaves][64];
    __shared__ float tx[1][kTbWaves][2];
    __shared__ int s_ok;
    const int nbytes = (int)((uint32_t)(A.nz + 2 * A.gz) * K.pbytes);
    const unsigned long long sbase = ((unsigned long long)A0.s_hi << 32) | A0.s_lo;
    const PrioQ pq(K.z0, K.z1 - K.z0 + 2);
    for (int t = 0; t < R0.npairs; ++t) {
        A.in = (t & 1) ? A0.out : A0.in;
        A.out = (t & 1) ? const_cast<float *>(A0.in) : A0.out;
        if (t > 0) A.fin = 1;
        K.rin = __builtin_amdgcn_make_buffer_rsrc((void *)A.in, (short)0, nbytes, 0x00020000);
        K.rout = __builtin_amdgcn_make_buffer_rsrc((void *)A.out, (short)0, nbytes, 0x00020000);
        const unsigned long long s0 = sbase + 2ull * (unsigned long long)t, s1 = s0 + 1;
        K.slo = (uint32_t)s0;
        K.shi = (uint32_t)(s0 >> 32);
        K.slo1 = (uint32_t)s1;
        K.shi1 = (uint32_t)(s1 >> 32);
        if (t > 0) {
            if (threadIdx.x == 0) {
                const bool ok = run_wait(R0, lb, A0.nyg, A0.nzc, R0.base + (unsigned int)t);
                if constexpr (LAUX == 0) {
                    __builtin_amdgcn_fence(__ATOMIC_ACQUIRE, "agent");
                    asm volatile("s_waitcnt vmcnt(0)" ::: "memory");
                }
                s_ok = ok ? 1 : 0;
            }
            __syncthreads();
            if (s_ok == 0) return;
        }
        if (R0.stamps != nullptr && threadIdx.x == 0) {
            R0.stamps[2 * ((size_t)t * nb + b)] = __builtin_amdgcn_s_memrealtime();
            if (t == 0)
                R0.stamps[2 * (size_t)R0.npairs * nb + b] =
                    ((unsigned long long)__builtin_amdgcn_s_getreg((20 << 0) | (0 << 6) | (31 << 11)) << 16) |
                    __builtin_amdgcn_s_getreg((4 << 0) | (0 << 6) | (31 << 11));
        }
        TbIn I0, I1, I2;
        {
            const __amdgpu_buffer_rsrc_t r0 = plane_rsrc(A.in, tb_pidx(A, K.z0 - 2), K.plane, K.pbytes);
            const __amdgpu_buffer_rsrc_t r1 = plane_rsrc(A.in, tb_pidx(A, K.z0 - 1), K.plane, K.pbytes);
            I0.row = bload4<LAUX>(r0, K.voff);
            I0.hm = I0.hp = I0.row;
            I1.row = bload4<LAUX>(r1, K.voff);
            I1.hm = bload4<LAUX>(r1, K.vm);
            I1.hp = bload4<LAUX>(r1, K.vp);
        }
        float4 T0 = make_float4(0.f, 0.f, 0.f, 0.f), T1 = T0, T2 = T0;
        FrameAcc f1 = frame_acc(), f2 = frame_acc();
        TbRun R;
        R.scur = (uint32_t)tb_pidx(A, K.z0 - 1) * K.pbytes;
        R.snext = (uint32_t)tb_pidx(A, K.z0) * K.pbytes;
        R.qz = (uint32_t)global_z(A, K.z0 - 1) * K.qplane;
        R.qzm = 0;
        const int z1 = K.z1;
        for (int p = K.z0 - 1; p <= z1; p += 3) {
            if (A.prio) prio_by_progress(pq.q(p));
            tb_plane<NZ, false, false, true, 0, false, LAUX>(A, K, R, p, I0, I1, I2, T0, T1, T2, lds, tx, f1, f2,
                                                             nullptr);
            if (p + 1 > z1) break;
            tb_plane<NZ, false, false, true, 1, false, LAUX>(A, K, R, p + 1, I1, I2, I0, T1, T2, T0, lds, tx, f1, f2,
                                                             nullptr);
            if (p + 2 > z1) break;
            tb_plane<NZ, false, false, true, 2, false, LAUX>(A, K, R, p + 2, I2, I0, I1, T2, T0, T1, lds, tx, f1, f2,
                                                             nullptr);
        }
        asm volatile("s_waitcnt vmcnt(0)" ::: "memory");
        __syncthreads();
        if (R0.stamps != nullptr && threadIdx.x == 0)
            R0.stamps[2 * ((size_t)t * nb + b) + 1] = __builtin_amdgcn_s_memrealtime();
        if (threadIdx.x == 0)
            __hip_atomic_store(R0.flags + lb, R0.base + (unsigned int)t + 1u, __ATOMIC_RELAXED,
                               __HIP_MEMORY_SCOPE_AGENT);
    }
}

template <bool NZ>
__global__ __launch_bounds__(kTbWaves * 64) __attribute__((amdgpu_waves_per_eu(1)))
void phi4_tb2_stage_kernel(const Phi4StepArgs A, const Tb2StageArgs S) {
    const int nb = gridDim.x, b = blockIdx.x;
    const TbBlock tbk = tb_block<false>(A, b, nb);
    const int Lx = A.Lx, Ly = A.Ly;
    TbCtx K;
    K.w = __builtin_amdgcn_readfirstlane((int)(threadIdx.x >> 6));
    K.lane = threadIdx.x & 63;
    K.outw = K.w >= 1 && K.w <= kTbRows;
    K.z0 = tbk.z0;
    K.z1 = tbk.z1;
    K.snapw = 0;
    K.plane = (size_t)Lx * (size_t)Ly;
    K.pbytes = (uint32_t)(K.plane * sizeof(float));
    K.qplane = (uint32_t)(K.plane >> 2);
    const int nbytes = (int)((uint32_t)(A.nz + 2 * A.gz) * K.pbytes);
    K.rin = __builtin_amdgcn_make_buffer_rsrc((void *)A.in, (short)0, nbytes, 0x00020000);
    K.rout = __builtin_amdgcn_make_buffer_rsrc((void *)A.out, (short)0, nbytes, 0x00020000);
    K.rstg = __builtin_amdgcn_make_buffer_rsrc((void *)S.stage, (short)0, (int)(2u * (uint32_t)S.G * K.pbytes),
                                               0x00020000);
    K.stg_g = S.G;
    K.stg_hi = A.nz - S.G;
    K.qwrap = (uint32_t)A.Lzg * K.qplane;
    K.m2v = f32x2{A.m2, A.m2};
    asm volatile("" : "+v"(K.m2v));
    K.swrap_at = INT_MIN;
    const unsigned long long s0 = ((unsigned long long)A.s_hi << 32) | A.s_lo, s1 = s0 + 1;
    K.slo = (uint32_t)s0;
    K.shi = (uint32_t)(s0 >> 32);
    K.slo1 = (uint32_t)s1;
    K.shi1 = (uint32_t)(s1 >> 32);
    {
        auto wrapy = [Ly](int y) { return y < 0 ? y + Ly : (y >= Ly ? y - Ly : y); };
        const int y = wrapy(tbk.yb * kTbRows - 1 + K.w);
        const int ym = wrapy(y - 1), yp = wrapy(y + 1);
        K.voff = (uint32_t)((y * Lx + 4 * K.lane) * 4);
        K.vm = (uint32_t)((ym * Lx + 4 * K.lane) * 4);
        K.vp = (uint32_t)((yp * Lx + 4 * K.lane) * 4);
        K.vex = 0;
        K.vx2 = 0;
        K.qoff = (uint32_t)((y * Lx + 4 * K.lane) >> 2);
    }
    __shared__ float4 lds[3][kTbWaves][64];
    __shared__ float tx[1][kTbWaves][2];
    TbIn I0, I1, I2;
    {
        const __amdgpu_buffer_rsrc_t r0 = plane_rsrc(A.in, tb_pidx(A, K.z0 - 2), K.plane, K.pbytes);
        const __amdgpu_buffer_rsrc_t r1 = plane_rsrc(A.in, tb_pidx(A, K.z0 - 1), K.plane, K.pbytes);
        I0.row = bload4(r0, K.voff);
        I0.hm = I0.hp = I0.row;
        I1.row = bload4(r1, K.voff);
        I1.hm = bload4(r1, K.vm);
        I1.hp = bload4(r1, K.vp);
    }
    float4 T0 = make_float4(0.f, 0.f, 0.f, 0.f), T1 = T0, T2 = T0;
    FrameAcc f1 = frame_acc(), f2 = frame_acc();
    TbRun R;
    R.scur = (uint32_t)tb_pidx(A, K.z0 - 1) * K.pbytes;
    R.snext = (uint32_t)tb_pidx(A, K.z0) * K.pbytes;
    R.qz = (uint32_t)global_z(A, K.z0 - 1) * K.qplane;
    R.qzm = 0;
    const int z1 = K.z1;
    const PrioQ pq(K.z0, z1 - K.z0 + 2);
    for (int p = K.z0 - 1; p <= z1; p += 3) {
        if (A.prio) prio_by_progress(pq.q(p));
        tb_plane<NZ, false, false, true, 0, false, 0, true>(A, K, R, p, I0, I1, I2, T0, T1, T2, lds, tx, f1, f2,
                                                            nullptr);
        if (p + 1 > z1) break;
        tb_plane<NZ, false, false, true, 1, false, 0, true>(A, K, R, p + 1, I1, I2, I0, T1, T2, T0, lds, tx, f1, f2,
                                                            nullptr);
        if (p + 2 > z1) break;
        tb_plane<NZ, false, false, true, 2, false, 0, true>(A, K, R, p + 2, I2, I0, I1, T2, T0, T1, lds, tx, f1, f2,
                                                            nullptr);
    }
    asm volatile("s_waitcnt vmcnt(0)" ::: "memory");
    __syncthreads();
    if (threadIdx.x == 0) __hip_atomic_fetch_add(S.ctr, 1u, __ATOMIC_RELAXED, __HIP_MEMORY_SCOPE_AGENT);
}

}

void phi4_run_kernel_id_name(uint64_t k, char *name, size_t cap) {
    if ((k >> 4) & 1)
        snprintf(name, cap, "phi4_tb2_stage_kernel<%s>", ((k >> 2) & 1) ? "true" : "false");
    else
        snprintf(name, cap, "phi4_tb2_run_kernel<%s, %d>", ((k >> 2) & 1) ? "true" : "false",
                 ((k >> 3) & 1) ? 16 : 0);
}

bool phi4_tb2_stage_ok(const Phi4StepArgs &a, int G) {
    return a.Lx == 256 && a.Ly % kTbRows == 0 && !a.periodic && a.nxseg == 1 && a.nyg == a.Ly / kTbRows &&
           a.nzr == a.nzc && a.nunits == a.nyg * a.nzc && a.zlo == 0 && a.zlen == a.nz && a.nz >= 2 &&
           (long long)a.zc * a.nzr >= a.zlen && G >= 1 && G <= a.nz && a.gz >= 2 && a.gate == nullptr &&
           a.flag == nullptr && a.st_md == nullptr && a.snap == nullptr && a.dcoef == nullptr &&
           a.stamps == nullptr && a.tctl == nullptr && a.fold.cin == nullptr && a.clr.md == nullptr &&
           (long long)(a.nz + 2 * a.gz) * a.Lx * a.Ly * 4 < (1ll << 31);
}

hipError_t phi4_tb2_stage_launch(const Phi4StepArgs &a, const Tb2StageArgs &g, hipStream_t s, hipEvent_t e0,
                                 hipEvent_t e1, uint64_t *kid) {
    if (!phi4_tb2_stage_ok(a, g.G) || g.stage == nullptr || g.ctr == nullptr) return hipErrorInvalidValue;
    const bool nz = a.sig != 0.0f;
    const dim3 grid((unsigned)a.nunits), block(kTbWaves * 64);
    if (kid != nullptr) *kid = (uint64_t)3 | (uint64_t)nz << 2 | (uint64_t)1 << 4 | (uint64_t)(grid.x * block.x) << 32;
    Phi4StepArgs q = a;
    static const int prio = getenv("SQ_TB2_PRIO") ? atoi(getenv("SQ_TB2_PRIO")) : 1;
    q.prio = prio;
    Tb2StageArgs gg = g;
    void *args[] = {&q, &gg};
    const void *fn = nz ? (const void *)&phi4_tb2_stage_kernel<true> : (const void *)&phi4_tb2_stage_kernel<false>;
    if (e0 != nullptr || e1 != nullptr) return hipExtLaunchKernel(fn, grid, block, args, 0, s, e0, e1, 0);
    return hipLaunchKernel(fn, grid, block, args, 0, s);
}

static int run_laux() {
    const char *e = getenv("SQ_TB2_RUN_SC1");
    return (e != nullptr && atoi(e) != 0) ? 16 : 0;
}

static const void *run_fn(bool nz, int laux) {
    if (laux == 16)
        return nz ? (const void *)&phi4_tb2_run_kernel<true, 16> : (const void *)&phi4_tb2_run_kernel<false, 16>;
    return nz ? (const void *)&phi4_tb2_run_kernel<true, 0> : (const void *)&phi4_tb2_run_kernel<false, 0>;
}

bool phi4_tb2_run_ok(const Phi4StepArgs &a, int dev) {
    if (a.Lx != 256 || a.Ly % kTbRows != 0 || !a.periodic || a.nxseg != 1 || a.nyg != a.Ly / kTbRows ||
        a.nzr != a.nzc || a.nunits != a.nyg * a.nzc || a.zlo != 0 || a.zlen != a.nz || a.zc < 2 ||
        a.zlen - (a.nzr - 1) * a.zc < 2 || (long long)a.zc * a.nzr < a.zlen)
        return false;
    if (a.gate != nullptr || a.flag != nullptr || a.st_md != nullptr || a.snap != nullptr || a.dcoef != nullptr ||
        a.stamps != nullptr || a.tctl != nullptr || a.fold.cin != nullptr || a.clr.md != nullptr)
        return false;
    if ((long long)(a.nz + 2 * a.gz) * a.Lx * a.Ly * 4 >= (1ll << 31)) return false;
    static int per_cu = -1, ncu = -1;
    if (per_cu < 0) {
        int n = 0;
        if (hipOccupancyMaxActiveBlocksPerMultiprocessor(&n, run_fn(true, 0), kTbWaves * 64, 0) != hipSuccess) n = 0;
        int c = 0;
        if (hipDeviceGetAttribute(&c, hipDeviceAttributeMultiprocessorCount, dev) != hipSuccess) c = 0;
        per_cu = n;
        ncu = c;
    }
    return (long long)a.nunits <= (long long)per_cu * ncu;
}

hipError_t phi4_tb2_run_launch(const Phi4StepArgs &a, const Tb2RunArgs &r, hipStream_t s, hipEvent_t e0,
                               hipEvent_t e1, uint64_t *kid) {
    if (r.npairs < 1 || r.flags == nullptr || r.err == nullptr) return hipErrorInvalidValue;
    const bool nz = a.sig != 0.0f;
    const int laux = run_laux();
    const dim3 grid((unsigned)a.nunits), block(kTbWaves * 64);
    if (kid != nullptr)
        *kid = (uint64_t)3 | (uint64_t)nz << 2 | (uint64_t)(laux == 16) << 3 | (uint64_t)(grid.x * block.x) << 32;
    Phi4StepArgs q = a;
    const char *pe = getenv("SQ_TB2_RUN_PRIO");
    q.prio = pe ? atoi(pe) : 1;
    Tb2RunArgs rr = r;
    void *args[] = {&q, &rr};
    const void *fn = run_fn(nz, laux);
    if (e0 != nullptr || e1 != nullptr) return hipExtLaunchKernel(fn, grid, block, args, 0, s, e0, e1, 0);
    return hipLaunchKernel(fn, grid, block, args, 0, s);
}

}
```

### stochquant_amd/csrc/sq_phi4_steps.cpp

```cpp
#include <algorithm>
#include <chrono>
#include <climits>
#include <cmath>
#include <cstdio>
#include <cstring>

#include "sq_ctx.h"

using namespace sq;

namespace {

sq::Phi4StepArgs phi4_base_args(sq_ctx *c, const Slab &s, int in_buf) {
    sq::Phi4StepArgs a{};
    a.in = s.buf[in_buf];
    a.out = s.buf[in_buf ^ 1];
    a.Lx = c->Lx;
    a.Ly = c->Ly;
    a.nz = s.nz;
    a.gz = c->gpad;
    a.zg0 = s.z0;
    a.Lzg = c->Lz;
    const float h = (float)c->dtau;
    a.h = h;
    a.m2 = (float)c->p.m2;
    a.lam6 = (float)((double)(float)c->p.lambda / 6.0);
    a.sig = (float)(sqrt(2.0 * (double)h) * c->p.C);
    a.sigq = (float)(sqrt(2.0 * (double)h) * c->p.C * sq::kSqrt2Ln2);
    a.fin = c->field_finite ? 1 : 0;
    a.clampv = (float)c->p.clamp;
    a.k0 = (uint32_t)c->p.seed;
    a.k1 = (uint32_t)(c->p.seed >> 32);
    a.s_lo = (uint32_t)c->step;
    a.s_hi = (uint32_t)(c->step >> 32);
    a.flag = c->in_frame ? c->flag : nullptr;
    a.st_md = nullptr;
    a.st_a = nullptr;
    a.dcoef = (c->in_frame && c->dev_frames) ? c->ctl_cur->coef : nullptr;
    if (c->in_frame && c->st_md != nullptr) {
        const size_t k = (size_t)(c->step - c->frame_step0) * sq::kStabSlots;
        a.st_md = c->st_md + k;
        a.st_a = c->st_a + k;
    }
    if (c->tri && c->in_frame) {
        a.buf0 = c->tri_bufs[0];
        a.buf1 = c->tri_bufs[1];
        a.buf2 = c->tri_bufs[2];
        a.tctl = c->ctl_cur;
        a.tk = c->frame_tk++;
        const int bi = a.tk == 0 ? c->spec_bs : ((a.tk & 1) ? c->spec_bw0 : c->spec_bw1);
        const int bo = a.tk == 0 ? c->spec_bw0 : ((a.tk & 1) ? c->spec_bw1 : c->spec_bw0);
        a.in = c->tri_bufs[bi];
        a.out = c->tri_bufs[bo];
        a.tspec = c->tri_spec ? 1 : 0;
    }
    return a;
}

int phi4_launch_range(sq_ctx *c, const Slab &s, int in_buf, hipStream_t st, int zlo, int zhi,
                      int zstep, int zc, int nzc, int periodic, bool timed) {
    if (nzc <= 0 || zhi <= zlo) return SQ_OK;
    sq::Phi4StepArgs a = phi4_base_args(c, s, in_buf);
    a.zlo = zlo;
    a.zhi = zhi;
    a.zstep = zstep;
    a.zc = zc;
    a.nzc = nzc;
    a.periodic = periodic;
    sq::phi4_fill_units(a, c->geom);
    EvPair *e = nullptr;
    if (timed && c->profiling == 1) {
        int rc = ev_take(c, &e);
        if (rc) return rc;
    }
    uint64_t kid = 0;
    SQ_HIP(sq::phi4_step_launch(a, c->geom, st, e ? e->a : nullptr, e ? e->b : nullptr, &kid));
    c->perf.kernel_launches += 1;
    c->kstat[kid] += 1;
    return SQ_OK;
}

int phi4_launch_span(sq_ctx *c, const Slab &s, int in_buf, hipStream_t st, int lo, int hi, bool timed) {
    if (hi <= lo) return SQ_OK;
    return phi4_launch_range(c, s, in_buf, st, lo, hi, c->zc, c->zc, (hi - lo + c->zc - 1) / c->zc, 0, timed);
}

void count_step(sq_ctx *c) {
    c->step += 1;
    c->perf.steps += 1;
    for (auto &s : c->slabs) c->perf.site_updates += (long long)s.nz * (long long)plane_floats(c);
}

constexpr int kRunUnsupported = -1000;

struct Tb2Opts {
    bool beside_xchg = false;
    hipEvent_t stop = nullptr;
    struct {
        bool on;
        int tlo0, thi0, tlen;
    } gate{false, 0, 0, 0};
    float *stage_slot = nullptr;
    int run_pairs = 0;
    bool stop_used = false;
    bool staged = false;
};

int phi4_tb2_range(sq_ctx *c, const Slab &s, int in_buf, hipStream_t st, int lo, int hi, int lo2, int hi2,
                   int periodic, bool timed, Tb2Opts &o) {
    if (hi <= lo) return SQ_OK;
    const int nr = lo2 < hi2 ? 2 : 1, len = hi - lo;
    if (nr == 2 && hi2 - lo2 != len) return fail(SQ_E_STATE, "two-step launch: ranges of different lengths");
    sq::Phi4StepArgs a = phi4_base_args(c, s, in_buf);
    a.snap = c->snap_next;
    c->snap_next = nullptr;
    a.stamps = c->stamps_next;
    c->stamps_next = nullptr;
    if (c->clr_armed) {
        a.clr = c->clr_next;
        c->clr_armed = false;
    }
    if (c->fold_next.cin != nullptr) {
        a.fold = c->fold_next;
        a.dcoef = nullptr;
        a.tctl = nullptr;
        c->fold_next = sq::FrameFoldArgs{};
        c->clr_armed = true;
    } else if (c->clr_first) {
        c->clr_armed = true;
    }
    c->clr_first = false;
    const int nyg = c->Ly / 8, nxseg = c->Lx / 256;
    const int target = o.beside_xchg ? c->tb_blocks_xchg : c->tb_blocks;
    const int nzc_t = std::max(1, target / (nyg * nxseg * (int)c->slabs.size() * nr));
    const int zb = c->tbz_pin ? c->tbz : std::min(len, std::max(c->tb_minz, (len + nzc_t - 1) / nzc_t));
    a.zlo = lo;
    a.zhi = nr == 2 ? hi2 : hi;
    a.zstep = nr == 2 ? lo2 - lo : 0;
    a.zc = zb;
    a.zlen = len;
    a.nzr = (len + zb - 1) / zb;
    a.nzc = nr * a.nzr;
    a.periodic = periodic;
    a.nxseg = nxseg;
    a.nyg = nyg;
    a.nunits = a.nxseg * a.nyg * a.nzc;
    if (o.gate.on) {
        a.gate = c->gate_word;
        a.gate_seq = c->gate_seq;
        a.gate_err = c->gate_err;
        a.n_reg = a.nunits;
        a.tzc = 4;
        a.tlen = o.gate.tlen;
        a.tlo0 = o.gate.tlo0;
        a.thi0 = o.gate.thi0;
        a.ntz = (a.tlen + a.tzc - 1) / a.tzc;
    }
    if (o.run_pairs > 0) {
        const int pairs = o.run_pairs;
        if (c->profiling == 1 || c->run_flags == nullptr || c->gate_err == nullptr || !sq::phi4_tb2_run_ok(a, c->dev))
            return kRunUnsupported;
        sq::Tb2RunArgs r{c->run_flags, c->gate_err, c->run_base, pairs, nullptr};
        const char *dpath = getenv("SQ_DIAG_RUN_STAMPS");
        const size_t nst = 2 * (size_t)pairs * a.nunits + a.nunits;
        if (dpath) SQ_HIP(hipMalloc(&r.stamps, nst * sizeof(unsigned long long)));
        uint64_t kid = 0;
        SQ_HIP(sq::phi4_tb2_run_launch(a, r, st, nullptr, nullptr, &kid));
        if (dpath) {
            std::vector<unsigned long long> h(nst + 2);
            h[0] = (unsigned long long)pairs;
            h[1] = (unsigned long long)a.nunits;
            SQ_HIP(hipStreamSynchronize(st));
            SQ_HIP(hipMemcpy(h.data() + 2, r.stamps, nst * sizeof(unsigned long long), hipMemcpyDeviceToHost));
            SQ_HIP(hipFree(r.stamps));
            if (FILE *f = fopen(dpath, "ab")) {
                fwrite(h.data(), sizeof(unsigned long long), h.size(), f);
                fclose(f);
            }
        }
        c->run_base += (unsigned int)pairs;
        c->perf.kernel_launches += 1;
        c->kstat[kid] += 1;
        c->perf.fused_steps += 2 * pairs;
        return SQ_OK;
    }
    EvPair *e = nullptr;
    if (timed && c->profiling == 1) {
        int rc = ev_take(c, &e);
        if (rc) return rc;
        c->ev_extra_steps += 1;
    }
    if (a.stamps != nullptr) {
        const int grid_n = a.nunits + (a.gate != nullptr ? a.nxseg * a.nyg * 2 * a.ntz : 0);
        if (grid_n > c->stamps_cap) return fail(SQ_E_STATE, "block stamps: more blocks than stamp slots");
        c->stamps_blocks = grid_n;
    }
    hipEvent_t stop = o.stop;
    uint64_t kid = 0;
    if (o.stage_slot != nullptr && stop == nullptr && sq::phi4_tb2_stage_ok(a, c->gz)) {
        const sq::Tb2StageArgs g{o.stage_slot, c->gz, c->kstage_ctr};
        SQ_HIP(sq::phi4_tb2_stage_launch(a, g, st, e ? e->a : nullptr, e ? e->b : nullptr, &kid));
        c->kstage_n += (unsigned int)a.nunits;
        o.staged = true;
    } else if (e == nullptr && stop != nullptr) {
        SQ_HIP(sq::phi4_tb2_launch(a, st, nullptr, stop, &kid));
        o.stop_used = true;
    } else {
        SQ_HIP(sq::phi4_tb2_launch(a, st, e ? e->a : nullptr, e ? e->b : nullptr, &kid));
    }
    c->perf.kernel_launches += 1;
    c->kstat[kid] += 1;
    c->perf.fused_steps += 2;
    return SQ_OK;
}

int phi4_tb2_pair(sq_ctx *c) {
    Slab &s = c->slabs[0];
    Tb2Opts o;
    int rc = phi4_tb2_range(c, s, c->cur, s.sA, 0, s.nz, 0, 0, 1, true, o);
    if (rc) return rc;
    c->cur ^= 1;
    count_step(c);
    count_step(c);
    return SQ_OK;
}

int phi4_tb2_run_pairs(sq_ctx *c, int pairs) {
    Slab &s = c->slabs[0];
    Tb2Opts o;
    o.run_pairs = pairs;
    int rc = phi4_tb2_range(c, s, c->cur, s.sA, 0, s.nz, 0, 0, 1, true, o);
    if (rc) return rc;
    c->cur ^= pairs & 1;
    for (int i = 0; i < 2 * pairs; ++i) count_step(c);
    return SQ_OK;
}

int phi4_periodic_step(sq_ctx *c) {
    Slab &s = c->slabs[0];
    const int nzc = (s.nz + c->zc - 1) / c->zc;
    int rc = phi4_launch_range(c, s, c->cur, s.sA, 0, s.nz, c->zc, c->zc, nzc, 1, true);
    if (rc) return rc;
    c->cur ^= 1;
    count_step(c);
    return SQ_OK;
}

int phi4_block(sq_ctx *c, int g) {
    const size_t plane = plane_floats(c);
    const int ns = (int)c->slabs.size(), G = c->gz;
    const size_t gbytes = (size_t)G * plane * sizeof(float);
    const int cur = c->cur;
    const unsigned long long step0 = c->step;
    std::vector<std::vector<sq_block_op>> plans;
    for (const Slab &s : c->slabs) plans.push_back(block_plan(s.nz, G, g, c->tbz > 0, c->edge_first, c->core_pairs, c->rims_b));
    std::vector<const float *> src_lo(ns), src_hi(ns);
    for (int i = 0; i < ns; ++i) {
        Slab &s = c->slabs[i];
        const float *p0 = plane0(c, s, cur);
        src_lo[i] = p0;
        src_hi[i] = p0 + (size_t)(s.nz - G) * plane;
    }
    const bool on_a = c->xchg_on_a && ns == 1 &&
                      ((c->p.comm == SQ_COMM_P2P && c->p2p_kernel_handshake) || c->p.comm == SQ_COMM_RCCL);
    const bool kst = c->p.comm == SQ_COMM_P2P && c->kstage_pending && ns == 1 && c->p2p_kernel_handshake &&
                     (on_a || c->kstage_env == 1);
    c->kstage_pending = false;
    for (int i = 0; i < ns; ++i) {
        Slab &s = c->slabs[i];
        if (kst || on_a) continue;
        if (c->evE_stale) {
            SQ_HIP(hipEventRecord(s.evE, s.sA));
            c->evE_stale = false;
        }
        if (!c->diag_no_ewait) SQ_HIP(hipStreamWaitEvent(s.sB, s.evE, 0));
        if (c->p.comm == SQ_COMM_LOOPBACK) {
            SQ_HIP(hipStreamWaitEvent(s.sB, c->slabs[(i + ns - 1) % ns].evE, 0));
            SQ_HIP(hipStreamWaitEvent(s.sB, c->slabs[(i + 1) % ns].evE, 0));
        }
    }
    const bool p2p = c->p.comm == SQ_COMM_P2P;
    if (p2p && !c->p2p_ready) return fail(SQ_E_STATE, "SQ_COMM_P2P context not connected (sq_p2p_connect)");
    const size_t slot_stride = 2 * (size_t)c->gpad * plane;
    const size_t slot = p2p ? (size_t)((c->xchg_seq + 1) & 1u) * slot_stride : 0;
    for (int i = 0; i < ns; ++i) {
        Slab &s = c->slabs[i];
        const bool staged_wait = plans[i][0].lo == 1;
        if (kst) continue;
        if (!staged_wait && !p2p) continue;
        if (!s.stage) return fail(SQ_E_STATE, "staged exchange without a staging buffer");
        float *stg = s.stage + slot;
        SQ_HIP(sq::p2p_copy2_launch(stg, src_lo[i], stg + (size_t)G * plane, src_hi[i], (size_t)G * plane,
                                    on_a ? s.sA : s.sB));
        if (staged_wait && !on_a) SQ_HIP(hipEventRecord(s.evS, s.sB));
        src_lo[i] = stg;
        src_hi[i] = stg + (size_t)G * plane;
    }
    if (c->p.comm == SQ_COMM_LOOPBACK) {
        for (int i = 0; i < ns; ++i) {
            Slab &s = c->slabs[i];
            Slab &dn = c->slabs[(i + ns - 1) % ns];
            Slab &up = c->slabs[(i + 1) % ns];
            SQ_HIP(hipMemcpyAsync(plane0(c, dn, cur) + (size_t)dn.nz * plane, src_lo[i], gbytes,
                                  hipMemcpyDeviceToDevice, s.sB));
            SQ_HIP(hipMemcpyAsync(plane0(c, up, cur) - (size_t)G * plane, src_hi[i], gbytes,
                                  hipMemcpyDeviceToDevice, s.sB));
            SQ_HIP(hipEventRecord(s.evC, s.sB));
            c->perf.halo_bytes += 2.0 * (double)gbytes;
        }
    } else if (p2p) {
        Slab &s = c->slabs[0];
        float *p0 = plane0(c, s, cur);
        const int P = c->p.nranks, r = c->p.rank;
        const int up = (r + 1) % P, dn = (r + P - 1) % P;
        const unsigned int e = ++c->xchg_seq;
        const size_t n = (size_t)G * plane;
        hipStream_t xs = on_a ? s.sA : s.sB;
        if (c->p2p_kernel_handshake) {
            SQ_HIP(sq::p2p_handshake_launch(c->peers[up].mbox + kMbStagedFromDn, c->peers[dn].mbox + kMbStagedFromUp,
                                            c->mbox + kMbStagedFromDn, c->mbox + kMbStagedFromUp, e,
                                            kHandshakePolls, c->gate_err, xs,
                                            (kst && !on_a) ? c->kstage_ctr : nullptr, c->kstage_n));
        } else {
            SQ_HIP(hipStreamWriteValue32(s.sB, c->peers[up].mbox + kMbStagedFromDn, e, 0));
            SQ_HIP(hipStreamWriteValue32(s.sB, c->peers[dn].mbox + kMbStagedFromUp, e, 0));
            SQ_HIP(wait_seq(s.sB, c->mbox + kMbStagedFromDn, e));
            SQ_HIP(wait_seq(s.sB, c->mbox + kMbStagedFromUp, e));
        }
        SQ_HIP(sq::p2p_copy2_launch(p0 - n, c->peers[dn].stage + slot + n, p0 + (size_t)s.nz * plane,
                                    c->peers[up].stage + slot, n, xs));
        if (!on_a) SQ_HIP(hipEventRecord(s.evC, s.sB));
        c->perf.halo_bytes += 2.0 * (double)gbytes;
    } else {
        Slab &s = c->slabs[0];
        float *p0 = plane0(c, s, cur);
        const int P = c->p.nranks, r = c->p.rank;
        const int up = (r + 1) % P, dn = (r + P - 1) % P;
        const size_t n = (size_t)G * plane;
        hipStream_t xs = on_a ? s.sA : s.sB;
        SQ_NCCLW(c, ncclGroupStart());
        SQ_NCCLW(c, ncclSend(src_hi[0], n, ncclFloat32, up, c->comm, xs));
        SQ_NCCLW(c, ncclSend(src_lo[0], n, ncclFloat32, dn, c->comm, xs));
        SQ_NCCLW(c, ncclRecv(p0 - n, n, ncclFloat32, dn, c->comm, xs));
        SQ_NCCLW(c, ncclRecv(p0 + (size_t)s.nz * plane, n, ncclFloat32, up, c->comm, xs));
        SQ_NCCLW(c, ncclGroupEnd());
        if (!on_a) SQ_HIP(hipEventRecord(s.evC, s.sB));
        c->perf.halo_bytes += 2.0 * (double)gbytes;
    }
    const bool gated = c->slab_gate && c->gate_word != nullptr && ns == 1 && per_rank(c->p.comm) &&
                       gate_pattern(plans[0]) >= 0;
    if (gated) SQ_HIP(hipStreamWriteValue32(c->slabs[0].sB, c->gate_word, ++c->gate_seq, 0));
    int out_buf = cur;
    bool stop_used = false;
    bool staged = false;
    for (int i = 0; i < ns; ++i) {
        Slab &s = c->slabs[i];
        const std::vector<sq_block_op> &ops = plans[i];
        std::vector<int> starts;
        for (const sq_block_op &op : ops)
            if (op.kind == SQ_OP_STEP || op.kind == SQ_OP_PAIR) starts.push_back(op.step);
        std::sort(starts.begin(), starts.end());
        starts.erase(std::unique(starts.begin(), starts.end()), starts.end());
        std::vector<char> timed(starts.size(), 0);
        bool xchg_live = true;
        for (size_t oi = 0; oi < ops.size(); ++oi) {
            const sq_block_op &op = ops[oi];
            int rc = SQ_OK;
            hipStream_t st = op.stream == kB ? s.sB : s.sA;
            Tb2Opts o;
            o.beside_xchg = xchg_live && op.stream != kB && c->p.comm != SQ_COMM_NONE;
            if (gated && (int)oi == gate_pattern(ops)) {
                const sq_block_op &rim = ops[oi + 2];
                const size_t gi = (size_t)(std::lower_bound(starts.begin(), starts.end(), op.step) - starts.begin());
                const int in = cur ^ (int)(gi & 1);
                const bool first = !timed[gi];
                timed[gi] = 1;
                c->step = step0 + (unsigned long long)op.step;
                o.gate = {true, rim.lo, rim.lo2, rim.hi - rim.lo};
                rc = phi4_tb2_range(c, s, in, st, op.lo, op.hi, 0, 0, 0, first, o);
                if (rc) return rc;
                xchg_live = false;
                oi += 2;
                continue;
            }
            if (op.kind == SQ_OP_STEP || op.kind == SQ_OP_PAIR) {
                const size_t gi = (size_t)(std::lower_bound(starts.begin(), starts.end(), op.step) - starts.begin());
                const int in = cur ^ (int)(gi & 1);
                const bool first = !timed[gi];
                timed[gi] = 1;
                c->step = step0 + (unsigned long long)op.step;
                stop_used = false;
                if (c->edges_stopev && op.kind == SQ_OP_PAIR && oi + 1 < ops.size() &&
                    ops[oi + 1].kind == SQ_OP_EDGES_DONE && ops[oi + 1].stream == op.stream)
                    o.stop = s.evE;
                staged = false;
                const bool kstage = p2p && kstage_on(c) && ns == 1 && c->p2p_kernel_handshake && !c->in_frame &&
                                     s.stage != nullptr && op.kind == SQ_OP_PAIR && op.stream == kA && op.lo == 0 &&
                                     op.hi == s.nz && op.lo2 >= op.hi2 && oi + 1 < ops.size() &&
                                     ops[oi + 1].kind == SQ_OP_EDGES_DONE && ops[oi + 1].stream == kA;
                if (kstage) o.stage_slot = s.stage + (size_t)((c->xchg_seq + 1) & 1u) * slot_stride;
                if (op.kind == SQ_OP_PAIR) {
                    rc = phi4_tb2_range(c, s, in, st, op.lo, op.hi, op.lo2, op.hi2, 0, first, o);
                    stop_used = o.stop_used;
                    staged = o.staged;
                } else if (op.lo2 < op.hi2)
                    rc = phi4_launch_range(c, s, in, st, op.lo, op.hi2, op.lo2 - op.lo, op.hi - op.lo, 2, 0, first);
                else
                    rc = phi4_launch_span(c, s, in, st, op.lo, op.hi, first);
            } else if (op.kind == SQ_OP_WAIT_EXCHANGE) {
                if (op.stream != kB) xchg_live = false;
                if (op.stream != kB && !c->diag_no_xwait && !on_a) SQ_HIP(hipStreamWaitEvent(st, s.evC, 0));
                if (c->p.comm == SQ_COMM_LOOPBACK) {
                    SQ_HIP(hipStreamWaitEvent(st, c->slabs[(i + ns - 1) % ns].evC, 0));
                    SQ_HIP(hipStreamWaitEvent(st, c->slabs[(i + 1) % ns].evC, 0));
                }
            } else if (op.kind == SQ_OP_WAIT_STAGED) {
                if (!kst) SQ_HIP(hipStreamWaitEvent(st, s.evS, 0));
            } else if (op.kind == SQ_OP_EDGES_DONE) {
                xchg_live = true;
                if (staged) {
                    c->kstage_pending = true;
                    c->evE_stale = true;
                    staged = false;
                } else if (on_a) {
                    c->evE_stale = true;
                } else if (!stop_used && !c->diag_no_ewait) {
                    SQ_HIP(hipEventRecord(s.evE, st));
                    c->evE_stale = false;
                }
                stop_used = false;
            } else if (op.kind == SQ_OP_SIGNAL || op.kind == SQ_OP_WAIT) {
                if (op.lo < 0 || op.lo >= kPlanSlots) return fail(SQ_E_STATE, "block op event slot out of range");
                if (op.kind == SQ_OP_SIGNAL)
                    SQ_HIP(hipEventRecord(s.evk[op.lo], st));
                else
                    SQ_HIP(hipStreamWaitEvent(st, s.evk[op.lo], 0));
            } else if (op.kind != SQ_OP_EXCHANGE) {
                return fail(SQ_E_STATE, "unknown block op");
            }
            if (rc) return rc;
        }
        out_buf = cur ^ (int)(starts.size() & 1);
    }
    c->step = step0;
    for (int k = 0; k < g; ++k) count_step(c);
    c->cur = out_buf;
    return SQ_OK;
}

int phi4_autotune(sq_ctx *c, int &n) {
    struct Cand {
        int g, k;
        bool rb, ef, a;
    };
    std::vector<Cand> cand;
    const bool ef = c->edge_first, a0 = c->xchg_on_a;
    for (int g : {4, 8, 16})
        if (g <= c->gpad) cand.push_back({g, c->core_pairs, c->rims_b, ef, a0});
    if (cand.empty()) cand.push_back({c->gpad, c->core_pairs, c->rims_b, ef, a0});
    const int gd = cand.back().g;
    if (c->tbz > 0 && c->k_auto && !a0) {
        cand.push_back({gd, 0, false, ef, false});
        for (bool rb : {false, true})
            for (int k : {2, 4})
                if (k <= gd / 2) cand.push_back({gd, k, rb, ef, false});
    }
    if (c->a_auto && !a0) cand.push_back({gd, 0, false, ef, true});
    if (c->ef_auto) cand.push_back({gd, c->core_pairs, c->rims_b, !ef, a0});
    if (cand.size() > 16) cand.resize(16);
    int need = 0;
    for (const Cand &k : cand) need += 3 * k.g;
    if (n < need) return SQ_OK;
    hipEvent_t t0, t1;
    SQ_HIP(hipEventCreate(&t0));
    SQ_HIP(hipEventCreate(&t1));
    std::vector<double> ms(cand.size());
    for (size_t k = 0; k < cand.size(); ++k) {
        const int g = cand[k].g;
        c->gz = g;
        c->core_pairs = cand[k].k;
        c->rims_b = cand[k].rb;
        c->edge_first = cand[k].ef;
        c->xchg_on_a = cand[k].a;
        int rc = phi4_block(c, g);
        if (!rc) rc = phi4_join(c);
        if (rc) return rc;
        SQ_HIP(hipEventRecord(t0, c->slabs[0].sA));
        for (int b = 0; b < 2 && !rc; ++b) rc = phi4_block(c, g);
        if (rc) return rc;
        SQ_HIP(hipEventRecord(t1, c->slabs[0].sA));
        SQ_HIP(hipEventSynchronize(t1));
        rc = phi4_join(c);
        if (rc) return rc;
        float e = 0;
        SQ_HIP(hipEventElapsedTime(&e, t0, t1));
        ms[k] = (double)e / (2.0 * g);
        n -= 3 * g;
    }
    (void)hipEventDestroy(t0);
    (void)hipEventDestroy(t1);
    if (per_rank(c->p.comm) && c->p.nranks > 1) {
        hipStream_t st = c->slabs[0].sA;
        SQ_HIP(hipMemcpyAsync(c->dtune, ms.data(), sizeof(double) * ms.size(), hipMemcpyHostToDevice, st));
        int rc = rank_allreduce(c, c->dtune, ms.size(), sq::P2pRed::kMaxF64, st);
        if (rc) return rc;
        SQ_HIP(hipMemcpyAsync(ms.data(), c->dtune, sizeof(double) * ms.size(), hipMemcpyDeviceToHost, st));
        SQ_HIP(hipStreamSynchronize(st));
    }
    const Cand best = cand[(size_t)sq_phi4_pick_ghost(ms.data(), (int)ms.size())];
    c->gz = best.g;
    c->core_pairs = best.k;
    c->rims_b = best.rb;
    c->edge_first = best.ef;
    c->xchg_on_a = best.a;
    c->g_tuned = true;
    return SQ_OK;
}

int phi4_steps_impl(sq_ctx *c, int n) {
    if (c->p.comm == SQ_COMM_NONE) {
        if (c->tb_run && c->tbz > 0 && n >= 4 && !c->in_frame && c->snap_next == nullptr &&
            c->stamps_next == nullptr && c->fold_next.cin == nullptr && !c->clr_armed && !c->clr_first) {
            int rc = gate_check(c, false);
            if (rc) return rc;
            const char *mp = getenv("SQ_TB2_RUN_MAXP");
            const int maxp = mp ? std::max(1, atoi(mp)) : INT_MAX;
            while (n >= 2) {
                const int np = std::min(n / 2, maxp);
                rc = phi4_tb2_run_pairs(c, np);
                if (rc == kRunUnsupported) {
                    c->tb_run = false;
                    break;
                }
                if (rc) return rc;
                n -= 2 * np;
            }
        }
        for (; c->tbz > 0 && n >= 2; n -= 2) {
            int rc = phi4_tb2_pair(c);
            if (rc) return rc;
        }
        for (int i = 0; i < n; ++i) {
            int rc = phi4_periodic_step(c);
            if (rc) return rc;
        }
        return SQ_OK;
    }
    if (c->p.comm == SQ_COMM_P2P && !c->p2p_ready)
        return fail(SQ_E_STATE, "SQ_COMM_P2P context not connected (sq_p2p_connect)");
    {
        int rc = fin_agree(c);
        if (rc) return rc;
    }
    if (c->g_auto && !c->g_tuned) {
        int rc = phi4_autotune(c, n);
        if (rc) return rc;
    }
    while (n > 0) {
        const int nb = (n + c->gz - 1) / c->gz;
        int g = (n + nb - 1) / nb;
        if (c->tbz > 0 && (g & 1) && g < c->gz) ++g;
        g = std::min(g, n);
        int rc = phi4_block(c, g);
        if (rc) return rc;
        n -= g;
    }
    return SQ_OK;
}

}

namespace sq {

bool kstage_on(const sq_ctx *c) { return c->kstage_env >= 0 ? c->kstage_env != 0 : c->xchg_on_a; }

int gate_check(sq_ctx *c, bool read_device) {
    if (!c->gate_failed && read_device && c->gate_err) {
        int e = 0;
        SQ_HIP(hipMemcpy(&e, c->gate_err, sizeof e, hipMemcpyDeviceToHost));
        if (e) c->gate_failed = true;
    }
    if (c->gate_failed)
        return fail(SQ_E_COMM, "slab exchange: gated rim chunks timed out waiting for the exchange, a P2P "
                               "hand-shake gave up waiting for a neighbour, or a resident march's block gave up "
                               "waiting for its neighbours (planes are stale; the field is corrupt until it is "
                               "uploaded or initialised again)");
    return SQ_OK;
}

int gate_reset(sq_ctx *c) {
    if (c->gate_err) SQ_HIP(hipMemset(c->gate_err, 0, sizeof(int)));
    if (c->run_flags) SQ_HIP(hipMemset(c->run_flags, 0, (size_t)c->run_nflags * sizeof(unsigned int)));
    c->kstage_pending = false;
    c->run_base = 0;
    c->gate_failed = false;
    return SQ_OK;
}

int fin_agree(sq_ctx *c) {
    if (!c->fin_sync) return SQ_OK;
    c->fin_sync = false;
    if (!per_rank(c->p.comm) || c->p.nranks <= 1) return SQ_OK;
    hipStream_t st = c->slabs[0].sA;
    double v = c->field_finite ? 0.0 : 1.0;
    SQ_HIP(hipMemcpyAsync(c->dtune, &v, sizeof v, hipMemcpyHostToDevice, st));
    int rc = rank_allreduce(c, c->dtune, 1, sq::P2pRed::kMaxF64, st);
    if (rc) return rc;
    SQ_HIP(hipMemcpyAsync(&v, c->dtune, sizeof v, hipMemcpyDeviceToHost, st));
    SQ_HIP(hipStreamSynchronize(st));
    c->field_finite = v == 0.0;
    return SQ_OK;
}

int phi4_steps(sq_ctx *c, int n) {
    const int rc = phi4_steps_impl(c, n);
    if (rc == SQ_OK && n > 0) c->field_finite = true;
    return rc;
}

int phi4_join(sq_ctx *c) {
    for (auto &s : c->slabs) {
        SQ_HIP(hipStreamSynchronize(s.sA));
        SQ_HIP(hipStreamSynchronize(s.sB));
    }
    return SQ_OK;
}

}

extern "C" {

int sq_step(sq_ctx *c, int nsteps) {
    if (!c) return fail(SQ_E_ARG, "null context");
    if (!is_phi4(c)) return fail(SQ_E_STATE, "sq_step is for PHI4 contexts (QM1D uses sq_run_frame)");
    if (nsteps < 0) return fail(SQ_E_ARG, "nsteps < 0");
    DeviceGuard g(c->dev);
    {
        int rc = gate_check(c, false);
        if (rc) return rc;
    }
    const auto t0 = std::chrono::steady_clock::now();
    EvPair *region = nullptr;
    if (c->profiling == 2 && nsteps > 0) {
        int rc = ev_take(c, &region);
        if (rc) return rc;
        SQ_HIP(hipEventRecord(region->a, c->slabs[0].sA));
    }
    {
        int rc = phi4_steps(c, nsteps);
        if (rc) return rc;
    }
    if (c->gate_err) {
        const char *ge = getenv("SQ_DIAG_GATE_ERR");
        if (ge && atoi(ge) != 0) SQ_HIP(hipMemsetAsync(c->gate_err, 1, 1, c->slabs[0].sA));
    }
    if (region) {
        SQ_HIP(hipEventRecord(region->b, c->slabs[0].sA));
        c->region_steps += nsteps;
    }
    c->perf.frame_ms += std::chrono::duration<double, std::milli>(std::chrono::steady_clock::now() - t0).count();
    return SQ_OK;
}

int sq_phi4_block_stamps(sq_ctx *c, unsigned long long *out, int cap, int *nblocks) {
    if (!c || !out || !nblocks || cap < 1) return fail(SQ_E_ARG, "null argument");
    if (!is_phi4(c)) return fail(SQ_E_STATE, "PHI4 only");
    if (c->slabs.size() != 1 || c->p.comm != SQ_COMM_NONE || c->tbz <= 0)
        return fail(SQ_E_STATE, "block stamps: one slab without an exchange, fused launches");
    DeviceGuard g(c->dev);
    const int need = std::max(cap, 4096);
    if (c->stamps_cap < need) {
        (void)hipFree(c->dstamps);
        c->stamps_cap = 0;
        SQ_HIP(hipMalloc(&c->dstamps, 4 * sizeof(unsigned long long) * (size_t)need));
        c->stamps_cap = need;
    }
    c->stamps_next = c->dstamps;
    c->stamps_blocks = 0;
    int rc = phi4_steps(c, 2);
    c->stamps_next = nullptr;
    if (rc) return rc;
    if (c->stamps_blocks > cap) return fail(SQ_E_ARG, "cap smaller than the launch's blocks");
    SQ_HIP(hipMemcpyAsync(out, c->dstamps, 2 * sizeof(unsigned long long) * (size_t)c->stamps_blocks,
                          hipMemcpyDeviceToHost, c->slabs[0].sA));
    SQ_HIP(hipStreamSynchronize(c->slabs[0].sA));
    *nblocks = c->stamps_blocks;
    return SQ_OK;
}

int sq_phi4_block_clocks(sq_ctx *c, unsigned long long *out, int cap, int *nblocks) {
    if (!c || !out || !nblocks || cap < 1) return fail(SQ_E_ARG, "null argument");
    if (!is_phi4(c)) return fail(SQ_E_STATE, "PHI4 only");
    if (c->dstamps == nullptr || c->stamps_blocks < 1) return fail(SQ_E_STATE, "no sq_phi4_block_stamps launch yet");
    if (c->stamps_blocks > cap) return fail(SQ_E_ARG, "cap smaller than the launch's blocks");
    DeviceGuard g(c->dev);
    const size_t n = 2 * (size_t)c->stamps_blocks;
    SQ_HIP(hipMemcpyAsync(out, c->dstamps + n, sizeof(unsigned long long) * n, hipMemcpyDeviceToHost,
                          c->slabs[0].sA));
    SQ_HIP(hipStreamSynchronize(c->slabs[0].sA));
    *nblocks = c->stamps_blocks;
    return SQ_OK;
}

}
```

### stochquant_amd/csrc/sq_rng.h

```cpp
#pragma once
#include <hip/hip_runtime.h>
#include <stdint.h>

namespace sq {

constexpr uint32_t kPhiloxM0 = 0xD2511F53u;
constexpr uint32_t kPhiloxM1 = 0xCD9E8D57u;
constexpr uint32_t kPhiloxW0 = 0x9E3779B9u;
constexpr uint32_t kPhiloxW1 = 0xBB67AE85u;

constexpr uint32_t kStreamField = 0;
constexpr uint32_t kStreamOmega = 1;
constexpr uint32_t kStreamInit = 2;

struct u32x4 {
    uint32_t x, y, z, w;
};

__device__ __forceinline__ u32x4 philox4x32_10(u32x4 c, uint32_t k0, uint32_t k1) {
#pragma unroll
    for (int r = 0; r < 10; ++r) {
        if (r) {
            k0 += kPhiloxW0;
            k1 += kPhiloxW1;
        }
        const uint64_t p0 = (uint64_t)kPhiloxM0 * c.x;
        const uint64_t p1 = (uint64_t)kPhiloxM1 * c.z;
        const uint32_t hi0 = (uint32_t)(p0 >> 32), lo0 = (uint32_t)p0;
        const uint32_t hi1 = (uint32_t)(p1 >> 32), lo1 = (uint32_t)p1;
        c = u32x4{hi1 ^ c.y ^ k0, lo1, hi0 ^ c.w ^ k1, lo0};
    }
    return c;
}

__device__ __forceinline__ u32x4 philox_counter(uint64_t quad, uint32_t stream, uint32_t step_lo,
                                                uint32_t step_hi) {
    return u32x4{(uint32_t)quad, ((uint32_t)(quad >> 32) & 0x00FFFFFFu) | (stream << 24), step_lo,
                 step_hi};
}

__device__ __forceinline__ float bm_u(uint32_t w0) { return 2.0f - __uint_as_float(0x3F800000u | (w0 & 0x007FFFFFu)); }
__device__ __forceinline__ float bm_t(uint32_t w1) { return __uint_as_float(0x3F800000u | (w1 & 0x007FFFFFu)); }
__device__ __forceinline__ float bm_radius(uint32_t w0) {
    return __builtin_amdgcn_sqrtf(__builtin_amdgcn_logf(bm_u(w0)) * -1.38629436111989061f);
}
__device__ __forceinline__ float bm_radius_q(uint32_t w0) {
    return __builtin_amdgcn_sqrtf(-__builtin_amdgcn_logf(bm_u(w0)));
}
__device__ __forceinline__ float bm_cos(uint32_t w1) { return __builtin_amdgcn_cosf(bm_t(w1)); }
__device__ __forceinline__ float bm_sin(uint32_t w1) { return __builtin_amdgcn_sinf(bm_t(w1)); }

__device__ __forceinline__ void box_muller(uint32_t w0, uint32_t w1, float &nc, float &ns) {
    const float r = bm_radius(w0);
    nc = r * bm_cos(w1);
    ns = r * bm_sin(w1);
}

__device__ __forceinline__ void box_muller_q(uint32_t w0, uint32_t w1, float &nc, float &ns) {
    const float r = bm_radius_q(w0);
    nc = r * bm_cos(w1);
    ns = r * bm_sin(w1);
}

struct f32x4n {
    float a, b, c, d;
};

__device__ __forceinline__ f32x4n normals4(uint64_t quad, uint32_t stream, uint32_t step_lo,
                                           uint32_t step_hi, uint32_t k0, uint32_t k1) {
    const u32x4 o = philox4x32_10(philox_counter(quad, stream, step_lo, step_hi), k0, k1);
    f32x4n n;
    box_muller(o.x, o.y, n.a, n.b);
    box_muller(o.z, o.w, n.c, n.d);
    return n;
}

}
```

Measured before the change: 1006 billion.

## Hoist step-invariant Philox rounds to host and reuse noise prefix across half-steps

Philox rounds that depend only on key, stream and step are precomputed on the host (or once per block) into per-step constants, so each site's noise runs a shorter per-lane prefix plus the remaining rounds. The second-half-step noise for plane z-1 reuses the prefix already computed for plane z in the first half-step, rekeyed through the inverse of the M1 multiplier, which avoids recomputing it. This adds carried NoisePre registers per plane slot, which may raise register pressure in a kernel that already loads several planes. Variants that cannot carry the prefix (wide with frames, and the run kernel) fall back to recomputing it.

After: 1025 billion (median of 6 runs). +1.9%, better.

```diff
diff --git a/stochquant_amd/build.py b/stochquant_amd/build.py
--- a/stochquant_amd/build.py
+++ b/stochquant_amd/build.py
@@ -23,7 +23,7 @@
 HOST_SOURCES = ["sq_core.cpp", "sq_comm.cpp", "sq_phi4_create.cpp", "sq_phi4_plan.cpp", "sq_phi4_steps.cpp",
                 "sq_phi4_frames.cpp", "sq_phi4_fields.cpp", "sq_qm1d_host.cpp", "sq_ens.cpp", "sq_phi4_ens.cpp",
                 "sq_diag.cpp", "sq_io.cpp"]
-HEADERS = ["sq_internal.h", "sq_ctx.h", "sq_rng.h", "sq_dpp.h", "sq_glibcf.h", "sq_ens.h", "sq_phi4_ens.h", "sq_qm1d_math.h"]
+HEADERS = ["sq_internal.h", "sq_ctx.h", "sq_rng.h", "sq_noise_consts.h", "sq_dpp.h", "sq_glibcf.h", "sq_ens.h", "sq_phi4_ens.h", "sq_qm1d_math.h"]
 INCLUDES = {"sq_phi4_run.hip": ["sq_phi4.hip"], "sq_phi4_ens.hip": ["sq_phi4.hip"]}
 COMMON = ["-O3", "-fPIC", "-std=c++17", "-ffp-contract=off", "-fno-slp-vectorize", "-Wall",
           "-Wno-unused-function"]
diff --git a/stochquant_amd/csrc/sq_internal.h b/stochquant_amd/csrc/sq_internal.h
--- a/stochquant_amd/csrc/sq_internal.h
+++ b/stochquant_amd/csrc/sq_internal.h
@@ -3,6 +3,8 @@
 #include <stdint.h>
 
 #include <string>
+
+#include "sq_noise_consts.h"
 
 namespace sq {
 
@@ -57,6 +59,7 @@
     float sigq;
     int fin;
     uint32_t k0, k1, s_lo, s_hi;
+    Phi4NoiseConsts nw0, nw1;
     int *flag;
     unsigned long long *st_md;
     unsigned int *st_a;
diff --git a/stochquant_amd/csrc/sq_noise_consts.h b/stochquant_amd/csrc/sq_noise_consts.h
--- /dev/null
+++ b/stochquant_amd/csrc/sq_noise_consts.h
@@ -0,0 +1,50 @@
+#pragma once
+#include <stdint.h>
+
+#if defined(__HIPCC__)
+#define SQ_HD __host__ __device__
+#else
+#define SQ_HD
+#endif
+
+namespace sq {
+
+constexpr uint32_t kPhiloxM0 = 0xD2511F53u;
+constexpr uint32_t kPhiloxM1 = 0xCD9E8D57u;
+constexpr uint32_t kPhiloxW0 = 0x9E3779B9u;
+constexpr uint32_t kPhiloxW1 = 0xBB67AE85u;
+constexpr uint32_t inv_u32(uint32_t a) {
+    uint32_t x = a;
+    for (int i = 0; i < 5; ++i) x *= 2u - a * x;
+    return x;
+}
+constexpr uint32_t kPhiloxM1Inv = inv_u32(kPhiloxM1);
+static_assert(kPhiloxM1 * kPhiloxM1Inv == 1u, "M1 inverse");
+
+constexpr uint32_t kStreamField = 0;
+constexpr uint32_t kStreamOmega = 1;
+constexpr uint32_t kStreamInit = 2;
+
+struct Phi4NoiseConsts {
+    uint32_t u0, u1, a0, b0, b2, u3, d2;
+};
+
+SQ_HD inline Phi4NoiseConsts phi4_noise_consts(uint32_t k0, uint32_t k1, uint64_t step) {
+    const uint32_t cy = kStreamField << 24, cz = (uint32_t)step, cw = (uint32_t)(step >> 32);
+    Phi4NoiseConsts w;
+    const uint64_t p1u = (uint64_t)kPhiloxM1 * cz;
+    w.u0 = (uint32_t)(p1u >> 32) ^ cy ^ k0;
+    w.u1 = (uint32_t)p1u;
+    w.a0 = cw ^ k1;
+    k0 += kPhiloxW0;
+    k1 += kPhiloxW1;
+    const uint64_t p0u = (uint64_t)kPhiloxM0 * w.u0;
+    w.b0 = w.u1 ^ k0;
+    w.b2 = (uint32_t)(p0u >> 32) ^ k1;
+    w.u3 = (uint32_t)p0u;
+    k1 += kPhiloxW1;
+    w.d2 = w.u3 ^ k1;
+    return w;
+}
+
+}
diff --git a/stochquant_amd/csrc/sq_phi4.hip b/stochquant_amd/csrc/sq_phi4.hip
--- a/stochquant_amd/csrc/sq_phi4.hip
+++ b/stochquant_amd/csrc/sq_phi4.hip
@@ -640,17 +640,13 @@
     int t0, t1, t2;
     __device__ __forceinline__ PrioQ(int z0, int span)
         : t0(z0 - 1 + (span + 3) / 4), t1(z0 - 1 + (2 * span + 3) / 4), t2(z0 - 1 + (3 * span + 3) / 4) {}
-    __device__ __forceinline__ int q(int p) const { return (p >= t0) + (p >= t1) + (p >= t2); }
+    __device__ __forceinline__ void set(int p) const {
+        if (p < t0) __builtin_amdgcn_s_setprio(3);
+        else if (p < t1) __builtin_amdgcn_s_setprio(2);
+        else if (p < t2) __builtin_amdgcn_s_setprio(1);
+        else __builtin_amdgcn_s_setprio(0);
+    }
 };
-
-__device__ __forceinline__ void prio_by_progress(int q) {
-    switch (q) {
-    case 0: __builtin_amdgcn_s_setprio(3); break;
-    case 1: __builtin_amdgcn_s_setprio(2); break;
-    case 2: __builtin_amdgcn_s_setprio(1); break;
-    default: __builtin_amdgcn_s_setprio(0); break;
-    }
-}
 
 struct TbBlock {
     int yb, xs, z0, z1;
@@ -723,6 +719,53 @@
     return xi;
 }
 
+struct NoisePre {
+    uint32_t h1, l1, n3;
+};
+
+__device__ __forceinline__ NoisePre noise_prefix(uint32_t quad, uint32_t a0) {
+    const uint64_t p0 = (uint64_t)kPhiloxM0 * quad;
+    const uint32_t n2 = (uint32_t)(p0 >> 32) ^ a0;
+    const uint64_t p1 = (uint64_t)kPhiloxM1 * n2;
+    return NoisePre{(uint32_t)(p1 >> 32), (uint32_t)p1, (uint32_t)p0};
+}
+
+__device__ __forceinline__ NoisePre noise_rekey(const NoisePre &q, uint32_t da) {
+    const uint32_t n2 = q.l1 * kPhiloxM1Inv;
+    const uint64_t p1 = (uint64_t)kPhiloxM1 * (n2 ^ da);
+    return NoisePre{(uint32_t)(p1 >> 32), (uint32_t)p1, q.n3};
+}
+
+template <bool NZ>
+__device__ __forceinline__ f32x4n tb_noise(const Phi4StepArgs &A, const NoisePre &q, const Phi4NoiseConsts &W) {
+    f32x4n xi;
+    if constexpr (NZ) {
+        uint32_t k0 = A.k0 + 2u * kPhiloxW0, k1 = A.k1 + 2u * kPhiloxW1;
+        u32x4 c;
+        {
+            const uint64_t p0 = (uint64_t)kPhiloxM0 * (q.h1 ^ W.b0);
+            const uint64_t p1 = (uint64_t)kPhiloxM1 * (W.b2 ^ q.n3);
+            const uint32_t n0 = __builtin_amdgcn_bitop3_b32((uint32_t)(p1 >> 32), q.l1, k0, 0x96);
+            c = u32x4{n0, (uint32_t)p1, (uint32_t)(p0 >> 32) ^ W.d2, (uint32_t)p0};
+        }
+#pragma unroll
+        for (int rnd = 3; rnd < 10; ++rnd) {
+            k0 += kPhiloxW0;
+            k1 += kPhiloxW1;
+            const uint64_t p0 = (uint64_t)kPhiloxM0 * c.x;
+            const uint64_t p1 = (uint64_t)kPhiloxM1 * c.z;
+            const uint32_t n0 = __builtin_amdgcn_bitop3_b32((uint32_t)(p1 >> 32), c.y, k0, 0x96);
+            const uint32_t m2 = __builtin_amdgcn_bitop3_b32((uint32_t)(p0 >> 32), c.w, k1, 0x96);
+            c = u32x4{n0, (uint32_t)p1, m2, (uint32_t)p0};
+        }
+        box_muller_q(c.x, c.y, xi.a, xi.b);
+        box_muller_q(c.z, c.w, xi.c, xi.d);
+    } else {
+        xi = f32x4n{0.f, 0.f, 0.f, 0.f};
+    }
+    return xi;
+}
+
 struct TbIn {
     float4 row, hm, hp;
 };
@@ -734,7 +777,8 @@
     uint32_t pbytes, qplane;
     __amdgpu_buffer_rsrc_t rin, rout;
     uint32_t voff, vm, vp, vex, vx2, qoff;
-    uint32_t slo, shi, slo1, shi1;
+    Phi4NoiseConsts nw0, nw1;
+    uint32_t da;
     uint32_t qwrap;
     f32x2 m2v;
     int swrap_at;
@@ -750,6 +794,12 @@
     uint32_t qz, qzm;
 };
 
+__device__ __forceinline__ void tb_noise_words(TbCtx &K, const Phi4NoiseConsts &w0, const Phi4NoiseConsts &w1) {
+    K.nw0 = w0;
+    K.nw1 = w1;
+    K.da = w0.a0 ^ w1.a0;
+}
+
 __device__ __forceinline__ float tb_site(float phi, float xm, float xp, float ym, float yp, float zm, float zp,
                                          float xi, const Phi4StepArgs &A, bool nz) {
     const float nb = ((xm + xp) + (ym + yp)) + (zm + zp);
@@ -771,10 +821,11 @@
     }
 }
 
-template <bool NZ, bool WIDE, bool FR, bool WH, int J, bool P2 = false, int LAUX = 0, bool STG = false>
+template <bool NZ, bool WIDE, bool FR, bool WH, int J, bool P2 = false, int LAUX = 0, bool STG = false, bool CY = true>
 __device__ __forceinline__ void tb_plane(const Phi4StepArgs &A, const TbCtx &K, TbRun &R, int p, const TbIn &I0,
                                          const TbIn &I1, TbIn &I2, const float4 &T0, const float4 &T1, float4 &T2,
-                                         float4 (*lds)[kTbWaves][64], float (*tx)[kTbWaves][2], FrameAcc &f1,
+                                         const NoisePre &Q1, NoisePre &Q2, float4 (*lds)[kTbWaves][64],
+                                         float (*tx)[kTbWaves][2], FrameAcc &f1,
                                          FrameAcc &f2, float *bmx, int *prog = nullptr) {
     constexpr int sl = J, sp = (J + 2) % 3;
     __amdgpu_buffer_rsrc_t rs, rc;
@@ -793,7 +844,8 @@
         I2.hp = bload4<LAUX>(rs, K.vp, ss);
         float ex = 0.f;
         if constexpr (WIDE) ex = bload1(rc, K.vex, sc);
-        const f32x4n xa = tb_noise<NZ>(A, R.qz, K.qoff, K.slo, K.shi);
+        const NoisePre qa = noise_prefix(R.qz + K.qoff, K.nw0.a0);
+        const f32x4n xa = tb_noise<NZ>(A, qa, K.nw0);
         float lft, rgt;
         if constexpr (WIDE) {
             lft = from_left_lane_or(I1.row.w, ex);
@@ -811,13 +863,17 @@
                     (f32x4v){I2.row.x, I2.row.y, I2.row.z, I2.row.w},
                     reinterpret_cast<f32x4v *>(reinterpret_cast<char *>(A.snap) + (size_t)(p + 1) * K.pbytes + K.voff));
         }
+        if constexpr (CY) {
+            Q2 = qa;
+            if (K.da != 0u) Q2 = noise_rekey(Q2, K.da);
+        }
         if constexpr (P2) tb_wait_nbrs(prog, K.w, p - 1);
         lds[sl][K.w][K.lane] = T2;
     } else {
         I2.row.x = bload1(rs, K.voff, ss);
         const float xm = bload1(rc, K.vex, sc), xp = bload1(rc, K.vx2, sc), ym = bload1(rc, K.vm, sc),
                     yp = bload1(rc, K.vp, sc);
-        const f32x4n n = tb_noise<NZ>(A, R.qz, K.qoff, K.slo, K.shi);
+        const f32x4n n = tb_noise<NZ>(A, noise_prefix(R.qz + K.qoff, K.nw0.a0), K.nw0);
         const float xi = K.lane >= 8 ? n.a : n.d;
         const float t = tb_site(I1.row.x, xm, xp, ym, yp, I0.row.x, I2.row.x, xi, A, NZ);
         if (K.lane < 16) tx[sl][(K.lane & 7) + 1][K.lane >> 3] = t;
@@ -828,7 +884,13 @@
         __syncthreads();
     }
     if (K.outw && p > K.z0) {
-        const f32x4n xb = tb_noise<NZ>(A, R.qzm, K.qoff, K.slo1, K.shi1);
+        NoisePre qb;
+        if constexpr (CY) {
+            qb = Q1;
+        } else {
+            qb = noise_prefix(R.qzm + K.qoff, K.nw1.a0);
+        }
+        const f32x4n xb = tb_noise<NZ>(A, qb, K.nw1);
         const float4 up = lds[sp][K.w - 1][K.lane], dn = lds[sp][K.w + 1][K.lane];
         float lft, rgt;
         if constexpr (WIDE) {
@@ -895,11 +957,7 @@
     K.m2v = f32x2{A.m2, A.m2};
     asm volatile("" : "+v"(K.m2v));
     K.swrap_at = A.periodic ? A.nz - 2 : INT_MIN;
-    const unsigned long long s0 = ((unsigned long long)A.s_hi << 32) | A.s_lo, s1 = s0 + 1;
-    K.slo = (uint32_t)s0;
-    K.shi = (uint32_t)(s0 >> 32);
-    K.slo1 = (uint32_t)s1;
-    K.shi1 = (uint32_t)(s1 >> 32);
+    tb_noise_words(K, A.nw0, A.nw1);
     const int xl = (x0 == 0 ? Lx : x0) - 1, xr = x0 + 256 == Lx ? 0 : x0 + 256;
     auto wrapy = [Ly](int y) { return y < 0 ? y + Ly : (y >= Ly ? y - Ly : y); };
     if (!WIDE || K.w < kTbWaves) {
@@ -957,6 +1015,7 @@
         }
     }
     float4 T0 = make_float4(0.f, 0.f, 0.f, 0.f), T1 = T0, T2 = T0;
+    NoisePre Q0{0u, 0u, 0u}, Q1 = Q0, Q2 = Q0;
     FrameAcc f1 = frame_acc(), f2 = frame_acc();
     __shared__ float bmx[2];
     __shared__ unsigned long long fk[2];
@@ -979,14 +1038,31 @@
         if (threadIdx.x < kTbWaves) prog[threadIdx.x] = K.z0 - 2;
         __syncthreads();
     }
+    constexpr bool CY = !WIDE && !FR;
     const PrioQ pq(K.z0, z1 - K.z0 + 2);
-    for (int p = K.z0 - 1; p <= z1; p += 3) {
-        if (A.prio) prio_by_progress(pq.q(p));
-        tb_plane<NZ, WIDE, FR, WH, 0, P2>(A, K, R, p, I0, I1, I2, T0, T1, T2, lds, tx, f1, f2, bmx, prog);
-        if (p + 1 > z1) break;
-        tb_plane<NZ, WIDE, FR, WH, 1, P2>(A, K, R, p + 1, I1, I2, I0, T1, T2, T0, lds, tx, f1, f2, bmx, prog);
-        if (p + 2 > z1) break;
-        tb_plane<NZ, WIDE, FR, WH, 2, P2>(A, K, R, p + 2, I2, I0, I1, T2, T0, T1, lds, tx, f1, f2, bmx, prog);
+    if constexpr (CY) {
+        for (int p = K.z0 - 1; p <= z1; p += 3) {
+            if (A.prio) pq.set(p);
+            tb_plane<NZ, WIDE, FR, WH, 0, P2>(A, K, R, p, I0, I1, I2, T0, T1, T2, Q1, Q2, lds, tx, f1, f2, bmx, prog);
+            if (p + 1 <= z1) {
+                tb_plane<NZ, WIDE, FR, WH, 1, P2>(A, K, R, p + 1, I1, I2, I0, T1, T2, T0, Q2, Q0, lds, tx, f1, f2, bmx, prog);
+                if (p + 2 <= z1)
+                    tb_plane<NZ, WIDE, FR, WH, 2, P2>(A, K, R, p + 2, I2, I0, I1, T2, T0, T1, Q0, Q1, lds, tx, f1, f2, bmx,
+                                                      prog);
+            }
+        }
+    } else {
+        for (int p = K.z0 - 1; p <= z1; p += 3) {
+            if (A.prio) pq.set(p);
+            tb_plane<NZ, WIDE, FR, WH, 0, P2, 0, false, false>(A, K, R, p, I0, I1, I2, T0, T1, T2, Q1, Q2, lds, tx, f1, f2, bmx,
+                                                               prog);
+            if (p + 1 > z1) break;
+            tb_plane<NZ, WIDE, FR, WH, 1, P2, 0, false, false>(A, K, R, p + 1, I1, I2, I0, T1, T2, T0, Q2, Q0, lds, tx, f1, f2,
+                                                               bmx, prog);
+            if (p + 2 > z1) break;
+            tb_plane<NZ, WIDE, FR, WH, 2, P2, 0, false, false>(A, K, R, p + 2, I2, I0, I1, T2, T0, T1, Q0, Q1, lds, tx, f1, f2,
+                                                               bmx, prog);
+        }
     }
     if constexpr (FR) frame_flush2(A, f1, f2, fk, fa);
     block_end_stamp(A);
@@ -1011,10 +1087,10 @@
     }
 }
 
-template <bool NZ, bool WIDE, bool FR, bool WH, int J>
+template <bool NZ, bool WIDE, bool FR, bool WH, int J, bool CY>
 __device__ __forceinline__ void tp_row(const Phi4StepArgs &A, const TbCtx &K, TpRun &R, int k, bool xrow,
-                                       uint32_t vxr, int xslot, float4 (&I)[4], float4 (&T)[4], float4 (&X)[2],
-                                       float (&E)[2], float4 (*in_lds)[kTpRows][64], float4 (*t_lds)[kTbWaves][64],
+                                       uint32_t vxr, int xslot, float4 (&I)[4], float4 (&T)[4], NoisePre (&Q)[4],
+                                       float4 (&X)[2], float (&E)[2], float4 (*in_lds)[kTpRows][64], float4 (*t_lds)[kTbWaves][64],
                                        float (*tx)[kTbWaves][2], FrameAcc &f1, FrameAcc &f2, float *bmx) {
     constexpr int im = J, ic = (J + 1) & 3, ip = (J + 2) & 3, in2 = (J + 3) & 3;
     constexpr int tc = J, tm = (J + 3) & 3, tmm = (J + 2) & 3;
@@ -1039,7 +1115,8 @@
         const bool sv = K.snapw != 0 && k + 1 >= K.z0 && k + 1 < K.z1;
         bstore4<2>(plane_rsrc(A.snap, k + 1, K.plane, K.pbytes), sv ? K.voff : kTpOob, I[ip]);
     }
-    const f32x4n xa = tb_noise<NZ>(A, R.qz, K.qoff, K.slo, K.shi);
+    const NoisePre qa = noise_prefix(R.qz + K.qoff, K.nw0.a0);
+    const f32x4n xa = tb_noise<NZ>(A, qa, K.nw0);
     const float4 up = in_lds[sc][K.w][K.lane], dn = in_lds[sc][K.w + 2][K.lane];
     float lft, rgt;
     if constexpr (WIDE) {
@@ -1054,11 +1131,21 @@
     if constexpr (FR) {
         if (K.outw && k >= K.z0 && k < K.z1) frame_sites<NZ, true>(A, f1, T[tc], I[ic], xa, bmx, true, mp1);
     }
+    if constexpr (CY) {
+        Q[tc] = qa;
+        if (K.da != 0u) Q[tc] = noise_rekey(Q[tc], K.da);
+    }
     t_lds[sc][K.w][K.lane] = T[tc];
     const bool bw = K.outw && k > K.z0;
     float4 o = T[tc];
     if (bw) {
-        const f32x4n xb = tb_noise<NZ>(A, R.qzm, K.qoff, K.slo1, K.shi1);
+        NoisePre qb;
+        if constexpr (CY) {
+            qb = Q[tm];
+        } else {
+            qb = noise_prefix(R.qzm + K.qoff, K.nw1.a0);
+        }
+        const f32x4n xb = tb_noise<NZ>(A, qb, K.nw1);
         const float4 bu = t_lds[sn][K.w - 1][K.lane], bd = t_lds[sn][K.w + 1][K.lane];
         float bl, br;
         if constexpr (WIDE) {
@@ -1104,7 +1191,7 @@
         NB[sn] = make_float4(bload1(r1, more ? K.vex : kTpOob, o1), bload1(r1, more ? K.vx2 : kTpOob, o1),
                              bload1(r1, more ? K.vm : kTpOob, o1), bload1(r1, more ? K.vp : kTpOob, o1));
     }
-    const f32x4n n = tb_noise<NZ>(A, R.qz, K.qoff, K.slo, K.shi);
+    const f32x4n n = tb_noise<NZ>(A, noise_prefix(R.qz + K.qoff, K.nw0.a0), K.nw0);
     const float xi = K.lane >= 8 ? n.a : n.d;
     const float t = tb_site(C[ic], NB[sc].x, NB[sc].y, NB[sc].z, NB[sc].w, C[im], C[ip], xi, A, NZ);
     if (K.lane < 16) tx[sc][(K.lane & 7) + 1][K.lane >> 3] = t;
@@ -1141,11 +1228,7 @@
     K.m2v = f32x2{A.m2, A.m2};
     asm volatile("" : "+v"(K.m2v));
     K.swrap_at = A.periodic ? A.nz : INT_MIN;
-    const unsigned long long s0 = ((unsigned long long)A.s_hi << 32) | A.s_lo, s1 = s0 + 1;
-    K.slo = (uint32_t)s0;
-    K.shi = (uint32_t)(s0 >> 32);
-    K.slo1 = (uint32_t)s1;
-    K.shi1 = (uint32_t)(s1 >> 32);
+    tb_noise_words(K, A.nw0, A.nw1);
     const int xl = (x0 == 0 ? Lx : x0) - 1, xr = x0 + 256 == Lx ? 0 : x0 + 256;
     auto wrapy = [Ly](int y) { return y < 0 ? y + Ly : (y >= Ly ? y - Ly : y); };
     const bool xw = WIDE && K.w == kTbWaves;
@@ -1200,6 +1283,7 @@
     const int z1 = K.z1;
     if (!xw) {
         float4 I[4], T[4], X[2];
+        NoisePre Q[4] = {};
         float E[2] = {0.f, 0.f};
         I[0] = bload4(p0, K.voff);
         I[1] = bload4(p1, K.voff);
@@ -1212,15 +1296,16 @@
         T[0] = T[1] = T[2] = T[3] = make_float4(0.f, 0.f, 0.f, 0.f);
         __syncthreads();
         const PrioQ pq(K.z0, z1 - K.z0 + 2);
+        constexpr bool CY = !(WIDE && FR && WPE == 6);
         for (int k = K.z0 - 1; k <= z1; k += 4) {
-            if (A.prio) prio_by_progress(pq.q(k));
-            tp_row<NZ, WIDE, FR, WH, 0>(A, K, R, k, xrow, vxr, xslot, I, T, X, E, in_lds, t_lds, tx, f1, f2, bmx);
+            if (A.prio) pq.set(k);
+            tp_row<NZ, WIDE, FR, WH, 0, CY>(A, K, R, k, xrow, vxr, xslot, I, T, Q, X, E, in_lds, t_lds, tx, f1, f2, bmx);
             if (k + 1 > z1) break;
-            tp_row<NZ, WIDE, FR, WH, 1>(A, K, R, k + 1, xrow, vxr, xslot, I, T, X, E, in_lds, t_lds, tx, f1, f2, bmx);
+            tp_row<NZ, WIDE, FR, WH, 1, CY>(A, K, R, k + 1, xrow, vxr, xslot, I, T, Q, X, E, in_lds, t_lds, tx, f1, f2, bmx);
             if (k + 2 > z1) break;
-            tp_row<NZ, WIDE, FR, WH, 2>(A, K, R, k + 2, xrow, vxr, xslot, I, T, X, E, in_lds, t_lds, tx, f1, f2, bmx);
+            tp_row<NZ, WIDE, FR, WH, 2, CY>(A, K, R, k + 2, xrow, vxr, xslot, I, T, Q, X, E, in_lds, t_lds, tx, f1, f2, bmx);
             if (k + 3 > z1) break;
-            tp_row<NZ, WIDE, FR, WH, 3>(A, K, R, k + 3, xrow, vxr, xslot, I, T, X, E, in_lds, t_lds, tx, f1, f2, bmx);
+            tp_row<NZ, WIDE, FR, WH, 3, CY>(A, K, R, k + 3, xrow, vxr, xslot, I, T, Q, X, E, in_lds, t_lds, tx, f1, f2, bmx);
         }
     } else {
         float C[4];
@@ -1232,7 +1317,7 @@
         __syncthreads();
         const PrioQ pq(K.z0, z1 - K.z0 + 2);
         for (int k = K.z0 - 1; k <= z1; k += 4) {
-            if (A.prio) prio_by_progress(pq.q(k));
+            if (A.prio) pq.set(k);
             tp_xhalo<NZ, WH, 0>(A, K, R, k, C, NB, tx);
             if (k + 1 > z1) break;
             tp_xhalo<NZ, WH, 1>(A, K, R, k + 1, C, NB, tx);
diff --git a/stochquant_amd/csrc/sq_phi4_run.hip b/stochquant_amd/csrc/sq_phi4_run.hip
--- a/stochquant_amd/csrc/sq_phi4_run.hip
+++ b/stochquant_amd/csrc/sq_phi4_run.hip
@@ -83,10 +83,7 @@
         K.rin = __builtin_amdgcn_make_buffer_rsrc((void *)A.in, (short)0, nbytes, 0x00020000);
         K.rout = __builtin_amdgcn_make_buffer_rsrc((void *)A.out, (short)0, nbytes, 0x00020000);
         const unsigned long long s0 = sbase + 2ull * (unsigned long long)t, s1 = s0 + 1;
-        K.slo = (uint32_t)s0;
-        K.shi = (uint32_t)(s0 >> 32);
-        K.slo1 = (uint32_t)s1;
-        K.shi1 = (uint32_t)(s1 >> 32);
+        tb_noise_words(K, phi4_noise_consts(A0.k0, A0.k1, s0), phi4_noise_consts(A0.k0, A0.k1, s1));
         if (t > 0) {
             if (threadIdx.x == 0) {
                 const bool ok = run_wait(R0, lb, A0.nyg, A0.nzc, R0.base + (unsigned int)t);
@@ -117,6 +114,7 @@
             I1.hp = bload4<LAUX>(r1, K.vp);
         }
         float4 T0 = make_float4(0.f, 0.f, 0.f, 0.f), T1 = T0, T2 = T0;
+        NoisePre Q0{0u, 0u, 0u}, Q1 = Q0, Q2 = Q0;
         FrameAcc f1 = frame_acc(), f2 = frame_acc();
         TbRun R;
         R.scur = (uint32_t)tb_pidx(A, K.z0 - 1) * K.pbytes;
@@ -125,15 +123,15 @@
         R.qzm = 0;
         const int z1 = K.z1;
         for (int p = K.z0 - 1; p <= z1; p += 3) {
-            if (A.prio) prio_by_progress(pq.q(p));
-            tb_plane<NZ, false, false, true, 0, false, LAUX>(A, K, R, p, I0, I1, I2, T0, T1, T2, lds, tx, f1, f2,
-                                                             nullptr);
+            if (A.prio) pq.set(p);
+            tb_plane<NZ, false, false, true, 0, false, LAUX, false, false>(A, K, R, p, I0, I1, I2, T0, T1, T2, Q1, Q2, lds, tx,
+                                                                           f1, f2, nullptr);
             if (p + 1 > z1) break;
-            tb_plane<NZ, false, false, true, 1, false, LAUX>(A, K, R, p + 1, I1, I2, I0, T1, T2, T0, lds, tx, f1, f2,
-                                                             nullptr);
+            tb_plane<NZ, false, false, true, 1, false, LAUX, false, false>(A, K, R, p + 1, I1, I2, I0, T1, T2, T0, Q2, Q0, lds,
+                                                                           tx, f1, f2, nullptr);
             if (p + 2 > z1) break;
-            tb_plane<NZ, false, false, true, 2, false, LAUX>(A, K, R, p + 2, I2, I0, I1, T2, T0, T1, lds, tx, f1, f2,
-                                                             nullptr);
+            tb_plane<NZ, false, false, true, 2, false, LAUX, false, false>(A, K, R, p + 2, I2, I0, I1, T2, T0, T1, Q0, Q1, lds,
+                                                                           tx, f1, f2, nullptr);
         }
         asm volatile("s_waitcnt vmcnt(0)" ::: "memory");
         __syncthreads();
@@ -172,11 +170,7 @@
     K.m2v = f32x2{A.m2, A.m2};
     asm volatile("" : "+v"(K.m2v));
     K.swrap_at = INT_MIN;
-    const unsigned long long s0 = ((unsigned long long)A.s_hi << 32) | A.s_lo, s1 = s0 + 1;
-    K.slo = (uint32_t)s0;
-    K.shi = (uint32_t)(s0 >> 32);
-    K.slo1 = (uint32_t)s1;
-    K.shi1 = (uint32_t)(s1 >> 32);
+    tb_noise_words(K, A.nw0, A.nw1);
     {
         auto wrapy = [Ly](int y) { return y < 0 ? y + Ly : (y >= Ly ? y - Ly : y); };
         const int y = wrapy(tbk.yb * kTbRows - 1 + K.w);
@@ -201,6 +195,7 @@
         I1.hp = bload4(r1, K.vp);
     }
     float4 T0 = make_float4(0.f, 0.f, 0.f, 0.f), T1 = T0, T2 = T0;
+    NoisePre Q0{0u, 0u, 0u}, Q1 = Q0, Q2 = Q0;
     FrameAcc f1 = frame_acc(), f2 = frame_acc();
     TbRun R;
     R.scur = (uint32_t)tb_pidx(A, K.z0 - 1) * K.pbytes;
@@ -210,15 +205,16 @@
     const int z1 = K.z1;
     const PrioQ pq(K.z0, z1 - K.z0 + 2);
     for (int p = K.z0 - 1; p <= z1; p += 3) {
-        if (A.prio) prio_by_progress(pq.q(p));
-        tb_plane<NZ, false, false, true, 0, false, 0, true>(A, K, R, p, I0, I1, I2, T0, T1, T2, lds, tx, f1, f2,
+        if (A.prio) pq.set(p);
+        tb_plane<NZ, false, false, true, 0, false, 0, true>(A, K, R, p, I0, I1, I2, T0, T1, T2, Q1, Q2, lds, tx, f1, f2,
                                                             nullptr);
-        if (p + 1 > z1) break;
-        tb_plane<NZ, false, false, true, 1, false, 0, true>(A, K, R, p + 1, I1, I2, I0, T1, T2, T0, lds, tx, f1, f2,
-                                                            nullptr);
-        if (p + 2 > z1) break;
-        tb_plane<NZ, false, false, true, 2, false, 0, true>(A, K, R, p + 2, I2, I0, I1, T2, T0, T1, lds, tx, f1, f2,
-                                                            nullptr);
+        if (p + 1 <= z1) {
+            tb_plane<NZ, false, false, true, 1, false, 0, true>(A, K, R, p + 1, I1, I2, I0, T1, T2, T0, Q2, Q0, lds, tx, f1, f2,
+                                                                nullptr);
+            if (p + 2 <= z1)
+                tb_plane<NZ, false, false, true, 2, false, 0, true>(A, K, R, p + 2, I2, I0, I1, T2, T0, T1, Q0, Q1, lds, tx, f1,
+                                                                    f2, nullptr);
+        }
     }
     asm volatile("s_waitcnt vmcnt(0)" ::: "memory");
     __syncthreads();
diff --git a/stochquant_amd/csrc/sq_phi4_steps.cpp b/stochquant_amd/csrc/sq_phi4_steps.cpp
--- a/stochquant_amd/csrc/sq_phi4_steps.cpp
+++ b/stochquant_amd/csrc/sq_phi4_steps.cpp
@@ -33,6 +33,8 @@
     a.k1 = (uint32_t)(c->p.seed >> 32);
     a.s_lo = (uint32_t)c->step;
     a.s_hi = (uint32_t)(c->step >> 32);
+    a.nw0 = sq::phi4_noise_consts(a.k0, a.k1, c->step);
+    a.nw1 = sq::phi4_noise_consts(a.k0, a.k1, c->step + 1);
     a.flag = c->in_frame ? c->flag : nullptr;
     a.st_md = nullptr;
     a.st_a = nullptr;
diff --git a/stochquant_amd/csrc/sq_rng.h b/stochquant_amd/csrc/sq_rng.h
--- a/stochquant_amd/csrc/sq_rng.h
+++ b/stochquant_amd/csrc/sq_rng.h
@@ -2,16 +2,9 @@
 #include <hip/hip_runtime.h>
 #include <stdint.h>
 
+#include "sq_noise_consts.h"
+
 namespace sq {
-
-constexpr uint32_t kPhiloxM0 = 0xD2511F53u;
-constexpr uint32_t kPhiloxM1 = 0xCD9E8D57u;
-constexpr uint32_t kPhiloxW0 = 0x9E3779B9u;
-constexpr uint32_t kPhiloxW1 = 0xBB67AE85u;
-
-constexpr uint32_t kStreamField = 0;
-constexpr uint32_t kStreamOmega = 1;
-constexpr uint32_t kStreamInit = 2;
 
 struct u32x4 {
     uint32_t x, y, z, w;
```
